# VolkmannB/bayesian-inference-with-explicit-and-implicit-prior-knowledge

Measured on AMD Instinct MI355X. Metric: particle-steps/sec (N x (T-1) / wall), SingleMassOscillator PGAS conditional-SMC sweep, higher is better.
Workload: dtype f64; 1 GPU; SingleMassOscillator PGAS sweep, nx=2, M=41 Hilbert basis (BASELINE.json configs[1]), N=1048576 particles/GPU, T=2000, fp64; particles_per_gpu=1048576, particles_total=1048576, T=2000, partition=single GPU, launch=every sweep enqueued launch by launch, verified=not checked in this run (--full checks the last timed sweep's traces), parallelism=1 GPU

## Files before the change

bayesian-inference-with-explicit-and-implicit-prior-knowledge_amd/_lib.py:

```python
from __future__ import annotations

import ctypes as C
import os

import numpy as np
import torch

_HERE = os.path.dirname(os.path.abspath(__file__))
LIB_PATH = os.environ.get("PGAS_HIP_LIB") or os.path.join(_HERE, "libpgas_hip.so")

_dp = C.POINTER(C.c_double)
_ip = C.POINTER(C.c_int32)


class PgasError(RuntimeError):
    pass


class _ModelDesc(C.Structure):
    _fields_ = [
        ("N", C.c_int32), ("T", C.c_int32), ("nx", C.c_int32), ("ny", C.c_int32), ("nu", C.c_int32),
        ("M", C.c_int32), ("D", C.c_int32),
        ("idx", _ip), ("sel", _ip), ("alpha", _dp), ("beta", _dp), ("nrm", C.c_double),
        ("H", _dp), ("LRinv", _dp), ("cR", C.c_double),
        ("m0", _dp), ("L0", _dp), ("y", _dp), ("u", _dp),
        ("device", C.c_int32), ("keep_logw_trace", C.c_int32), ("no_fast_variant", C.c_int32),
    ]


EXPORTS = [
    "pgas_create", "pgas_destroy", "pgas_last_error", "pgas_segment_size", "pgas_set_params", "pgas_set_params_dev", "pgas_get_params", "pgas_basis_eval",
    "pgas_aux_states", "pgas_init_state", "pgas_step", "pgas_sweep", "pgas_get_traces", "pgas_last_final_index",
    "pgas_suffstats", "pgas_set_profiling", "pgas_get_profile", "pgas_set_option",
    "pgas_systematic_resample", "pgas_reconstruct_trajectory",
    "pgas_trace_layout", "pgas_trace_row",
    "pgas_shard_setup", "pgas_shard_buffers", "pgas_shard_layout", "pgas_shard_block", "pgas_shard_set_peer_block", "pgas_shard_run", "pgas_ipc_export", "pgas_ipc_open",
    "pgas_hip_runtime_version", "pgas_shard_unique_id", "pgas_shard_comm_init", "pgas_shard_sweep", "pgas_shard_set_collective", "pgas_get_launch_info", "pgas_shard_probe_collective", "pgas_detmath_eval",
    "pgas_m_rng_uniform", "pgas_m_rng_normal", "pgas_m_rng_student_t", "pgas_m_rng_student_t_host", "pgas_m_rng_chi2", "pgas_m_set_time_source", "pgas_m_rng_uniform_dev", "pgas_systematic_resample_dev", "pgas_m_mniw_solve", "pgas_m_mniw_trisolve", "pgas_m_check", "pgas_m_stats_gather_update", "pgas_m_weighted_stats",
    "pgas_m_mniw_solve_n", "pgas_m_mniw_trisolve_n", "pgas_m_stats_gather_update_n", "pgas_m_weighted_stats_n", "pgas_m_expr_eval",
    "pgas_m_rng_student_t_df", "pgas_m_mniw_draw", "pgas_m_hilbert_basis", "pgas_m_lbm_diff",
    "pgas_chains_set_params_dev", "pgas_chains_sweep", "pgas_chains_get_traces", "pgas_chains_final_index", "pgas_chains_keys",
    "pgas_chains_param_draws", "pgas_chains_suffstats", "pgas_rollout", "pgas_rollout_stats", "pgas_filter",
    "pgas_m_runs_rng_normal", "pgas_m_runs_rng_student_t", "pgas_m_runs_rng_student_t_df", "pgas_m_runs_rng_uniform", "pgas_m_runs_systematic",
    "pgas_m_runs_weighted_stats", "pgas_m_rollout", "pgas_m_rollout_stats",
]



class RolloutLatent(C.Structure):
    _fields_ = [("M", C.c_int32), ("D", C.c_int32), ("n", C.c_int32), ("feat", C.c_int32), ("sel", C.c_int32 * 4),
                ("div", C.c_double * 4), ("center", C.c_double * 4), ("L", C.c_double * 4), ("size", C.c_double * 4),
                ("idx_dev", C.c_void_p), ("A_dev", C.c_void_p), ("Lrow_dev", C.c_void_p), ("fcode_dev", C.c_void_p), ("fcode_host", C.c_void_p),
                ("f_ninstr", C.c_int32), ("reserved", C.c_int32)]


class RolloutDesc(C.Structure):
    _fields_ = [(k, C.c_int32) for k in ("K", "T", "P", "L", "nx", "nu", "ny", "n_in", "nconst", "nreg", "x0_mode", "f_ninstr", "g_ninstr", "reserved")] + \
               [("f_out", C.c_int32 * 8), ("g_out", C.c_int32 * 8), ("p0", C.c_int64)] + \
               [(k, C.c_void_p) for k in ("consts_dev", "fcode_dev", "gcode_dev", "fcode_host", "gcode_host", "inputs_dev", "seeds_dev", "Qc_dev", "x0_dev",
                                          "m0L0_dev", "out_x_dev", "out_y_dev")] + \
               [("lat", RolloutLatent * 4)]


class RolloutStatsDesc(C.Structure):
    _fields_ = [(k, C.c_void_p) for k in ("y_dev", "sum_dev", "sumsq_dev", "lpd_dev", "part_dev")] + \
               [("part_bytes", C.c_uint64), ("cR", C.c_double), ("noise", C.c_int32), ("reserved", C.c_int32), ("LR", C.c_double * 64), ("LRinv", C.c_double * 64)]


ALLGATHER_FN = C.CFUNCTYPE(C.c_int, C.c_void_p, C.c_int32, C.c_void_p)

_lib = None


def load():
    global _lib
    if _lib is not None:
        return _lib
    if not os.path.exists(LIB_PATH):
        raise PgasError(f"{LIB_PATH} not found: build it with `python __graft_entry__.py` (hipcc, gfx950); there is no CPU fallback")
    L = C.CDLL(LIB_PATH)

    class _Missing:
        restype = argtypes = None

        def __init__(self, name):
            self.name = name

        def __call__(self, *a):
            raise PgasError(f"{LIB_PATH} does not export {self.name}")

    for name in EXPORTS:
        if not hasattr(L, name):
            setattr(L, name, _Missing(name))
    vp, u64, i32, i64 = C.c_void_p, C.c_uint64, C.c_int32, C.c_int64
    L.pgas_create.restype = C.c_int
    L.pgas_create.argtypes = [C.POINTER(_ModelDesc), C.POINTER(vp)]
    L.pgas_destroy.restype = None
    L.pgas_destroy.argtypes = [vp]
    L.pgas_last_error.restype = C.c_char_p
    L.pgas_last_error.argtypes = [vp]
    L.pgas_segment_size.restype = i32
    L.pgas_set_params.restype = C.c_int
    L.pgas_set_params.argtypes = [vp, vp, _dp, _dp, C.c_double, vp]
    L.pgas_set_params_dev.restype = C.c_int
    L.pgas_set_params_dev.argtypes = [vp, vp, vp, vp]
    L.pgas_get_params.restype = C.c_int
    L.pgas_get_params.argtypes = [vp, _dp, _dp, _dp, vp]
    L.pgas_basis_eval.restype = C.c_int
    L.pgas_basis_eval.argtypes = [vp, vp, i64, i32, vp, vp]
    L.pgas_aux_states.restype = C.c_int
    L.pgas_aux_states.argtypes = [vp, vp, i32, vp, vp]
    L.pgas_init_state.restype = C.c_int
    L.pgas_init_state.argtypes = [vp, u64, _dp, vp, vp]
    L.pgas_step.restype = C.c_int
    L.pgas_step.argtypes = [vp, i32, u64, vp, vp, _dp, vp, vp, vp, vp]
    L.pgas_sweep.restype = C.c_int
    L.pgas_sweep.argtypes = [vp, u64, vp, vp, vp]
    L.pgas_get_traces.restype = C.c_int
    L.pgas_get_traces.argtypes = [vp, C.POINTER(vp), C.POINTER(vp), C.POINTER(vp), C.POINTER(vp)]
    L.pgas_last_final_index.restype = C.c_int
    L.pgas_last_final_index.argtypes = [vp, C.POINTER(i64), vp]
    L.pgas_suffstats.restype = C.c_int
    L.pgas_suffstats.argtypes = [vp, vp, vp, vp, vp, vp]
    L.pgas_set_profiling.restype = C.c_int
    L.pgas_set_profiling.argtypes = [vp, i32]
    L.pgas_get_profile.restype = C.c_int
    L.pgas_get_profile.argtypes = [vp, C.POINTER(i64), C.POINTER(C.c_double), C.POINTER(i64), C.POINTER(C.c_double), vp]
    L.pgas_set_option.restype = C.c_int
    L.pgas_set_option.argtypes = [vp, i32, i64]
    L.pgas_systematic_resample.restype = C.c_int
    L.pgas_systematic_resample.argtypes = [vp, C.c_double, vp, vp, vp]
    L.pgas_reconstruct_trajectory.restype = C.c_int
    L.pgas_reconstruct_trajectory.argtypes = [vp, vp, vp, i32, i32, i64, vp, vp]
    L.pgas_shard_setup.restype = C.c_int
    L.pgas_shard_setup.argtypes = [vp, i32, i32]
    L.pgas_shard_buffers.restype = C.c_int
    L.pgas_shard_buffers.argtypes = [vp, C.POINTER(vp), C.POINTER(i64)]
    L.pgas_shard_layout.restype = C.c_int
    L.pgas_shard_layout.argtypes = [vp, i32, C.POINTER(i64)]
    L.pgas_shard_block.restype = C.c_int
    L.pgas_shard_block.argtypes = [vp, i32, i32, C.POINTER(vp), C.POINTER(i64)]
    L.pgas_shard_set_peer_block.restype = C.c_int
    L.pgas_shard_set_peer_block.argtypes = [vp, i32, i32, i32, vp]
    L.pgas_trace_layout.restype = C.c_int
    L.pgas_trace_layout.argtypes = [vp, i32, C.POINTER(i64)]
    L.pgas_trace_row.restype = C.c_int
    L.pgas_trace_row.argtypes = [vp, i32, i32, C.POINTER(vp)]
    L.pgas_shard_run.restype = C.c_int
    L.pgas_shard_run.argtypes = [vp, i32, i32, i32, u64, vp, vp, vp]
    L.pgas_shard_unique_id.restype = C.c_int
    L.pgas_shard_unique_id.argtypes = [C.c_char_p]
    L.pgas_shard_comm_init.restype = C.c_int
    L.pgas_shard_comm_init.argtypes = [vp, C.c_char_p]
    L.pgas_shard_sweep.restype = C.c_int
    L.pgas_shard_sweep.argtypes = [vp, u64, vp, vp, i32, vp]
    L.pgas_shard_set_collective.restype = C.c_int
    L.pgas_shard_set_collective.argtypes = [vp, ALLGATHER_FN, vp]
    L.pgas_detmath_eval.restype = C.c_int
    L.pgas_detmath_eval.argtypes = [i32, i32, vp, vp, vp, i64, vp, vp, vp, vp]
    L.pgas_shard_probe_collective.restype = C.c_int
    L.pgas_shard_probe_collective.argtypes = [vp, i32, vp]
    L.pgas_get_launch_info.restype = C.c_int
    L.pgas_get_launch_info.argtypes = [vp, C.POINTER(i32)]
    L.pgas_ipc_export.restype = C.c_int
    L.pgas_ipc_export.argtypes = [vp, i32, i32, C.c_char_p]
    L.pgas_hip_runtime_version.restype = C.c_int32
    L.pgas_hip_runtime_version.argtypes = []
    L.pgas_ipc_open.restype = C.c_int
    L.pgas_ipc_open.argtypes = [vp, C.c_char_p, C.POINTER(vp)]
    u32 = C.c_uint32
    L.pgas_m_rng_uniform.restype = C.c_double
    L.pgas_m_rng_uniform.argtypes = [u64, u32, u32]
    L.pgas_m_rng_normal.restype = C.c_int
    L.pgas_m_rng_normal.argtypes = [vp, u64, u32, u32, i64, i64, i32, vp, vp]
    L.pgas_m_rng_student_t.restype = C.c_int
    L.pgas_m_rng_student_t.argtypes = [vp, u64, u32, u32, i64, i64, vp, vp, vp]
    L.pgas_m_rng_student_t_host.restype = C.c_int
    L.pgas_m_rng_student_t_host.argtypes = [u64, u32, u32, i64, i64, _dp, _dp]
    L.pgas_m_set_time_source.restype = C.c_int
    L.pgas_m_set_time_source.argtypes = [vp, vp]
    L.pgas_m_rng_uniform_dev.restype = C.c_int
    L.pgas_m_rng_uniform_dev.argtypes = [vp, u64, u32, u32, vp, vp]
    L.pgas_systematic_resample_dev.restype = C.c_int
    L.pgas_systematic_resample_dev.argtypes = [vp, vp, vp, vp, vp]
    L.pgas_m_rng_chi2.restype = C.c_int
    L.pgas_m_rng_chi2.argtypes = [vp, u64, u32, u32, i64, i64, vp, vp, vp]
    L.pgas_m_mniw_solve.restype = C.c_int
    L.pgas_m_mniw_solve.argtypes = [vp, i64, i32, C.c_double, vp, vp, vp, vp, vp, vp, vp, vp, vp, vp, vp, vp, vp, vp]
    L.pgas_m_mniw_trisolve.restype = C.c_int
    L.pgas_m_mniw_trisolve.argtypes = [vp, i64, i32, vp, vp, vp, vp, vp, vp]
    L.pgas_m_rng_student_t_df.restype = C.c_int
    L.pgas_m_rng_student_t_df.argtypes = [vp, u64, C.c_uint32, C.c_uint32, i64, i64, vp, vp, C.c_double, C.c_double, vp, vp]
    L.pgas_m_mniw_draw.restype = C.c_int
    L.pgas_m_mniw_draw.argtypes = [vp, i64, C.c_double, vp, vp, vp, vp, vp, vp, C.c_double, C.c_double, vp, vp, vp]
    L.pgas_m_lbm_diff.restype = C.c_int
    L.pgas_m_lbm_diff.argtypes = [vp, i64, i32, vp, vp, vp, vp, vp, vp, C.c_double, C.c_double, vp, vp, vp, vp]
    L.pgas_m_hilbert_basis.restype = C.c_int
    L.pgas_m_hilbert_basis.argtypes = [vp, i64, i32, i32, vp, i32, vp, i32, C.POINTER(i32), _dp, _dp, _dp, _dp, vp, vp, vp]
    L.pgas_m_expr_eval.restype = C.c_int
    L.pgas_m_expr_eval.argtypes = [vp, i64, vp, i32, vp, i32, i32, i32, C.POINTER(i32), i32, vp, i32, vp, vp, i32, C.POINTER(vp), C.POINTER(i32), i32, i32,
                                   vp, vp, C.c_double, vp, vp]
    L.pgas_m_mniw_solve_n.restype = C.c_int
    L.pgas_m_mniw_solve_n.argtypes = [vp, i64, i32, i32, C.c_double, vp, vp, vp, vp, vp, vp, vp, vp, vp, vp, vp, vp, vp, vp]
    L.pgas_m_mniw_trisolve_n.restype = C.c_int
# ... 155 lines not shown
    def get_params(self):
        LS, LSinv, cS = np.zeros((self.nx, self.nx)), np.zeros((self.nx, self.nx)), C.c_double()
        self._chk(self.lib.pgas_get_params(self._h, _hp(LS), _hp(LSinv), C.byref(cS), self._stream()), "pgas_get_params")
        return LS, LSinv, float(cS.value)

    def basis_eval(self, x, t):
        x = self._dev(x).reshape(-1, self.nx)
        phi = torch.empty((x.shape[0], self.M), dtype=torch.float64, device=self.device)
        self._chk(self.lib.pgas_basis_eval(self._h, x.data_ptr(), x.shape[0], t, phi.data_ptr(), self._stream()), "pgas_basis_eval")
        return phi

    def aux_states(self, x, t):
        x = self._dev(x, shape=(self.N, self.nx))
        aux = torch.empty_like(x)
        self._chk(self.lib.pgas_aux_states(self._h, x.data_ptr(), t, aux.data_ptr(), self._stream()), "pgas_aux_states")
        return aux

    def init_state(self, seed, ref0):
        x0 = torch.empty((self.N, self.nx), dtype=torch.float64, device=self.device)
        r = _f64(ref0).reshape(self.nx)
        self._chk(self.lib.pgas_init_state(self._h, seed, _hp(r), x0.data_ptr(), self._stream()), "pgas_init_state")
        torch.cuda.current_stream(self.device).synchronize()
        return x0

    def step(self, t, seed, log_weights, state, ref_t):
        x = self._dev(state, shape=(self.N, self.nx))
        lw = None if log_weights is None else self._dev(log_weights, shape=(self.N,))
        r = _f64(ref_t.detach().cpu() if isinstance(ref_t, torch.Tensor) else ref_t).reshape(self.nx)
        lw_new = torch.empty(self.N, dtype=torch.float64, device=self.device)
        x_new = torch.empty((self.N, self.nx), dtype=torch.float64, device=self.device)
        anc = torch.empty(self.N, dtype=torch.int32, device=self.device)
        self._chk(
            self.lib.pgas_step(self._h, t, seed, None if lw is None else lw.data_ptr(), x.data_ptr(), _hp(r), lw_new.data_ptr(),
                               x_new.data_ptr(), anc.data_ptr(), self._stream()),
            "pgas_step",
        )
        torch.cuda.current_stream(self.device).synchronize()
        return lw_new, x_new, anc

    def sweep(self, seed, ref_state):
        ref = self._dev(ref_state, shape=(self.T, self.nx))
        traj = torch.empty((self.T, self.nx), dtype=torch.float64, device=self.device)
        self._chk(self.lib.pgas_sweep(self._h, seed, ref.data_ptr(), traj.data_ptr(), self._stream()), "pgas_sweep")
        self._ref_keepalive = ref
        return traj

    TRACE_X, TRACE_LA, TRACE_H, TRACE_LN, TRACE_ANC = range(5)

    def trace_layout(self, kind):
        v = (C.c_int64 * 4)()
        self._chk(self.lib.pgas_trace_layout(self._h, int(kind), v), "pgas_trace_layout")
        return tuple(int(x) for x in v)

    def trace_row(self, kind, t):
        p = C.c_void_p()
        self._chk(self.lib.pgas_trace_row(self._h, int(kind), int(t), C.byref(p)), "pgas_trace_row")
        return int(p.value)

    def traces_blocks(self, kind, row_shape, dtype):
        rows, rpb, nblk, _ = self.trace_layout(kind)
        return [self.dev_tensor(self.trace_row(kind, b * rpb), (min(rpb, rows - b * rpb),) + tuple(row_shape), dtype) for b in range(nblk)]

    def traces(self, copy_blocks=True):
        px, pa, pl, pt = C.c_void_p(), C.c_void_p(), C.c_void_p(), C.c_void_p()
        if self.trace_layout(self.TRACE_X)[2] == 1 and self.trace_layout(self.TRACE_ANC)[2] == 1:
            px.value, pa.value = self.trace_row(self.TRACE_X, 0), self.trace_row(self.TRACE_ANC, 0)
            X = torch.as_tensor(_DevView(px.value, (self.T, self.N, self.nx), "<f8", self), device=self.device)
            A = torch.as_tensor(_DevView(pa.value, (max(self.T - 1, 1), self.N), "<i4", self), device=self.device)
        elif copy_blocks:
            X = torch.cat(self.traces_blocks(self.TRACE_X, (self.N, self.nx), torch.float64))
            A = torch.cat(self.traces_blocks(self.TRACE_ANC, (self.N,), torch.int32))
        else:
            X = A = None
        self._chk(self.lib.pgas_get_traces(self._h, None, None, C.byref(pl), C.byref(pt)), "pgas_get_traces")
        Lw = torch.as_tensor(_DevView(pl.value, (self.N,), "<f8", self), device=self.device)
        Lt = torch.as_tensor(_DevView(pt.value, (self.T, self.N), "<f8", self), device=self.device) if pt.value else None
        return X, A, Lw, Lt

    def last_final_index(self):
        v = C.c_int64()
        self._chk(self.lib.pgas_last_final_index(self._h, C.byref(v), self._stream()), "pgas_last_final_index")
        return int(v.value)

    def set_profiling(self, on):
        self._chk(self.lib.pgas_set_profiling(self._h, int(on)), "pgas_set_profiling")

    def profile(self):
        n, ms, pn, pm = C.c_int64(), C.c_double(), C.c_int64(), C.c_double()
        self._chk(self.lib.pgas_get_profile(self._h, C.byref(n), C.byref(ms), C.byref(pn), C.byref(pm), self._stream()), "pgas_get_profile")
        return int(n.value), float(ms.value), int(pn.value), float(pm.value)

    def set_option(self, option, value):
        self._chk(self.lib.pgas_set_option(self._h, int(option), int(value)), "pgas_set_option")

    _utility = {}

    @classmethod
    def utility(cls, N, device=None):
        from .descriptors import BasisMap, GaussianLikelihood, HilbertBasis

        dev = torch.device("cuda", torch.cuda.current_device()) if device is None else torch.device(device)
        key = (dev.index or 0, int(N))
        if key not in cls._utility:
            basis = HilbertBasis(np.array([[1]], dtype=np.int32), np.array([[-1.0, 1.0]]))
            cls._utility[key] = cls(int(N), np.zeros((1, 1)), None, np.zeros(1), np.eye(1), GaussianLikelihood(np.eye(1), np.eye(1)),
                                    BasisMap(basis, [0]), device=dev)
        return cls._utility[key]

    def systematic_resample(self, u, logw):
        lw = self._dev(logw, shape=(self.N,))
        idx = torch.empty(self.N, dtype=torch.int32, device=self.device)
        if isinstance(u, torch.Tensor):
            self._chk(self.lib.pgas_systematic_resample_dev(self._h, u.data_ptr(), lw.data_ptr(), idx.data_ptr(), self._stream()), "pgas_systematic_resample_dev")
        else:
            self._chk(self.lib.pgas_systematic_resample(self._h, float(u), lw.data_ptr(), idx.data_ptr(), self._stream()), "pgas_systematic_resample")
        return idx

    def reconstruct_trajectory(self, particles, ancestry, idx):
        P = particles if isinstance(particles, torch.Tensor) else torch.as_tensor(np.asarray(particles, dtype=np.float64))
        P = P.to(device=self.device, dtype=torch.float64)
        if P.dim() == 2:
            P = P.unsqueeze(-1)
        P = P.contiguous()
        T, N, nx = P.shape
        if N != self.N:
            raise ValueError(f"particle count {N} does not match the context ({self.N})")
        A = ancestry if isinstance(ancestry, torch.Tensor) else torch.as_tensor(np.asarray(ancestry))
        A = A.to(device=self.device, dtype=torch.int32).contiguous()
        traj = torch.empty((T, nx), dtype=torch.float64, device=self.device)
        self._chk(self.lib.pgas_reconstruct_trajectory(self._h, P.data_ptr(), A.data_ptr(), T, nx, int(idx), traj.data_ptr(), self._stream()),
                  "pgas_reconstruct_trajectory")
        return traj

    def shard_setup(self, rank, world):
        self._chk(self.lib.pgas_shard_setup(self._h, rank, world), "pgas_shard_setup")
        self.rank, self.world = rank, world

    def shard_buffers(self):
        out = (C.c_void_p * 17)()
        sz = (C.c_int64 * 3)()
        self._chk(self.lib.pgas_shard_buffers(self._h, out, sz), "pgas_shard_buffers")
        return [int(p or 0) for p in out], tuple(int(v) for v in sz)

    def shard_layout(self, which):
        v = (C.c_int64 * 2)()
        self._chk(self.lib.pgas_shard_layout(self._h, int(which), v), "pgas_shard_layout")
        return int(v[0]), int(v[1])

    def shard_block(self, which, blk):
        p, n = C.c_void_p(), C.c_int64()
        self._chk(self.lib.pgas_shard_block(self._h, int(which), int(blk), C.byref(p), C.byref(n)), "pgas_shard_block")
        return int(p.value), int(n.value)

    def shard_set_peer_block(self, peer, which, blk, ptr):
        self._chk(self.lib.pgas_shard_set_peer_block(self._h, int(peer), int(which), int(blk), C.c_void_p(int(ptr))), "pgas_shard_set_peer_block")

    def shard_run(self, phase, t=0, t_aux=0, seed=0, ref=None, traj=None):
        self._chk(
            self.lib.pgas_shard_run(self._h, phase, t, t_aux, seed, None if ref is None else ref.data_ptr(),
                                    None if traj is None else traj.data_ptr(), self._stream()),
            "pgas_shard_run",
        )

    def shard_unique_id(self):
        buf = C.create_string_buffer(128)
        rc = self.lib.pgas_shard_unique_id(buf)
# ... 455 lines not shown
```

bayesian-inference-with-explicit-and-implicit-prior-knowledge_amd/csrc/pgas_api.hip:

```cpp
#include <hip/hip_runtime.h>
#include <hip/hip_ext.h>
#include <dlfcn.h>
#include <rccl/rccl.h>

#include <algorithm>
#include <cmath>
#include <cstdio>
#include <cstdlib>
#include <cstring>
#include <string>
#include <vector>

#include "../../include/pgas_hip.h"
#include "pgas_kernels.hip.h"
#include "pgas_resample.hip.h"
#include "pgas_suffstats.hip.h"
#include "pgas_marginal.hip.h"
#include "pgas_marginal_runs.hip.h"
#include "pgas_chains.hip.h"
#include "pgas_rollout.hip.h"
#include "pgas_rollout_stats.hip.h"
#include "pgas_filter.hip.h"
#include "../../include/pgas_marginal.h"
#include "pgas_marginal_rollout.hip.h"
// ... 230 lines not shown
    int force_slow = 0;
    int tail_groups = 0;
    int ev_stride = 8;
    int local_groups = 0;
    int overlap = 1;
    int prop_lds = 0;
    hipStream_t sB = nullptr;
    std::vector<hipEvent_t> ev_chunk;
    hipEvent_t ev_start = nullptr, ev_done = nullptr;
    double* d_phi = nullptr;
    double* d_syrk_ws = nullptr;
    size_t phi_bytes = 0, syrk_ws_bytes = 0;
    int syrk_splits = 0;
    bool peer_access_tried = false;
    const uint32_t* t_dev = nullptr;
    int max_lead = 0;
    std::vector<hipEvent_t> ev_bdone;
    int profiling = 0;
    int prof_stride = 16;
    std::vector<hipEvent_t> ev;
    std::vector<hipEvent_t> evp;
    int evp_used = 0;
    int ev_used = 0;
    int ch_cap = 0;
    int ch_params = 0;
    int ch_swept = 0;
    TransParams* ch_tp = nullptr;
    double* ch_G = nullptr;
    SweepParams* ch_sp = nullptr;
    double* ch_ures = nullptr;
    double* ch_uanc = nullptr;
    double* ch_x = nullptr;
    int32_t* ch_anc = nullptr;
    double* ch_logw = nullptr;
    UpperHdr* ch_hdr = nullptr;
    double* ch_znoise = nullptr;
    int ro_cap = 0;
    TransParams* ro_tp = nullptr;
    double* ro_G = nullptr;
    double* ro_S0 = nullptr;
    double* ro_part = nullptr;
    size_t ro_part_cap = 0;
    int fl_cap = 0;
    TransParams* fl_tp = nullptr;
    double* fl_G = nullptr;
    std::string err;
};

#define FAIL(ctx, code, ...)                                  \
    do {                                                      \
        char buf_[512];                                       \
        snprintf(buf_, sizeof buf_, __VA_ARGS__);             \
        (ctx)->err = buf_;                                    \
        return (code);                                        \
    } while (0)

#define HIPCHK(ctx, call)                                                                       \
    do {                                                                                        \
        hipError_t e_ = (call);                                                                 \
        if (e_ != hipSuccess) FAIL(ctx, e_ == hipErrorOutOfMemory ? PGAS_E_NOMEM : PGAS_E_HIP,  \
                                   "%s failed: %s", #call, hipGetErrorString(e_));              \
    } while (0)

#define KCHK(ctx, name)                                                                        \
    do {                                                                                        \
        hipError_t e_ = hipGetLastError();                                                      \
        if (e_ != hipSuccess) FAIL(ctx, PGAS_E_HIP, "launch of %s failed: %s", name, hipGetErrorString(e_)); \
    } while (0)

static int alloc_scanbufs(pgas_ctx* c, ScanBufs* sb) {
    const size_t np = (size_t)c->md.nseg * PGAS_SEG;
    const int nsegp = (c->md.nseg + 63) / 64 * 64;
    sb->nsegp = nsegp;
    HIPCHK(c, hipMalloc(&sb->laux, np * sizeof(double)));
    HIPCHK(c, hipMalloc(&sb->c1, np * sizeof(uint64_t)));
    HIPCHK(c, hipMalloc(&sb->c2, np * sizeof(uint64_t)));
    HIPCHK(c, hipMalloc(&sb->segk_w, 2 * nsegp * sizeof(double)));
    HIPCHK(c, hipMalloc(&sb->segs_w, 2 * nsegp * sizeof(uint64_t)));
    HIPCHK(c, hipMalloc(&sb->tab_e, 2 * nsegp * sizeof(double)));
    HIPCHK(c, hipMalloc(&sb->tab_sc, 2 * nsegp * sizeof(double)));
    HIPCHK(c, hipMalloc(&sb->tab_m, 2 * nsegp * sizeof(double)));
    HIPCHK(c, hipMalloc(&sb->grp_K, 2 * PG_MAX_GRP * sizeof(double)));
    HIPCHK(c, hipMalloc(&sb->grp_T, 2 * PG_MAX_GRP * sizeof(double)));
    HIPCHK(c, hipMalloc(&sb->grp_cnt, PG_MAX_GRP * sizeof(unsigned)));
    HIPCHK(c, hipMemset(sb->grp_cnt, 0, PG_MAX_GRP * sizeof(unsigned)));
    HIPCHK(c, hipMalloc(&sb->hdr, sizeof(UpperHdr)));
    HIPCHK(c, hipMemset(sb->hdr, 0, sizeof(UpperHdr)));
    sb->segk = sb->segk_w;
    sb->segs = sb->segs_w;
    sb->nseg_l = 0x40000000;
    sb->rank_stride = 0;
    sb->nsegp_g = nsegp;
    return PGAS_OK;
}
static void chains_release(pgas_ctx* c) {
    hipFree(c->ch_tp); hipFree(c->ch_G); hipFree(c->ch_sp); hipFree(c->ch_ures); hipFree(c->ch_uanc); hipFree(c->ch_x); hipFree(c->ch_anc);
    hipFree(c->ch_logw); hipFree(c->ch_hdr); hipFree(c->ch_znoise);
    c->ch_tp = nullptr; c->ch_G = nullptr; c->ch_sp = nullptr; c->ch_ures = nullptr; c->ch_uanc = nullptr; c->ch_x = nullptr; c->ch_anc = nullptr;
    c->ch_logw = nullptr; c->ch_hdr = nullptr; c->ch_znoise = nullptr;
    c->ch_cap = c->ch_params = c->ch_swept = 0;
}
static void rollout_release(pgas_ctx* c) {
    hipFree(c->ro_tp); hipFree(c->ro_G); hipFree(c->ro_S0);
    c->ro_tp = nullptr; c->ro_G = nullptr; c->ro_S0 = nullptr;
    c->ro_cap = 0;
}
static void rollout_part_release(pgas_ctx* c) {
    hipFree(c->ro_part);
    c->ro_part = nullptr;
    c->ro_part_cap = 0;
}
static void filter_release(pgas_ctx* c) {
    hipFree(c->fl_tp); hipFree(c->fl_G);
    c->fl_tp = nullptr; c->fl_G = nullptr;
    c->fl_cap = 0;
}
static void free_scanbufs(ScanBufs* sb) {
    hipFree(sb->laux); hipFree(sb->c1); hipFree(sb->c2); hipFree(sb->segk_w); hipFree(sb->segs_w);
    hipFree(sb->tab_e); hipFree(sb->tab_sc); hipFree(sb->tab_m); hipFree(sb->grp_K); hipFree(sb->grp_T); hipFree(sb->grp_cnt); hipFree(sb->hdr);
    *sb = ScanBufs{};
}

extern "C" {

int32_t pgas_segment_size(void) { return PGAS_SEG; }

const char* pgas_last_error(const pgas_ctx* ctx) { return ctx ? ctx->err.c_str() : g_create_error.c_str(); }

static int create_impl(const pgas_model_desc* d, pgas_ctx* c) {
    if (!d->idx || !d->sel || !d->alpha || !d->beta || !d->H || !d->LRinv || !d->m0 || !d->L0 || !d->y)
        FAIL(c, PGAS_E_ARG, "pgas_create: NULL table pointer");
    if (d->N < 1 || d->T < 1 || d->M < 1) FAIL(c, PGAS_E_ARG, "pgas_create: N, T, M must be >= 1");
    if (d->nx < 1 || d->nx > 2) FAIL(c, PGAS_E_ARG, "pgas_create: nx = %d not supported (compiled for nx in {1,2})", d->nx);
    if (d->ny < 1 || d->ny > PGAS_MAX_NY) FAIL(c, PGAS_E_ARG, "pgas_create: ny = %d not supported (1..%d)", d->ny, PGAS_MAX_NY);
    if (d->nu < 0 || d->nu > PGAS_MAX_NU) FAIL(c, PGAS_E_ARG, "pgas_create: nu = %d not supported (0..%d)", d->nu, PGAS_MAX_NU);
    if (d->D < 1 || d->D > PGAS_MAX_D) FAIL(c, PGAS_E_ARG, "pgas_create: D = %d not supported (1..%d)", d->D, PGAS_MAX_D);
    if (d->nu > 0 && !d->u) FAIL(c, PGAS_E_ARG, "pgas_create: nu > 0 but u == NULL");
    const int64_t nseg64 = ((int64_t)d->N + PGAS_SEG - 1) / PGAS_SEG;
    if (nseg64 > PG_MAX_NSEG) FAIL(c, PGAS_E_ARG, "pgas_create: N = %d exceeds %d particles per device", d->N, PG_MAX_NSEG * PGAS_SEG);

    DevModel& md = c->md;
    md.N = d->N; md.T = d->T; md.nx = d->nx; md.ny = d->ny; md.nu = d->nu; md.D = d->D; md.M = d->M;
    md.nseg = (int)nseg64;
    md.p0 = 0; md.Ng = d->N; md.nseg_g = md.nseg;
    c->peers = Peers{}; c->peers.world = 1; c->peers.nseg_l = md.nseg; c->peers.Nl = d->N;
    md.nrm = d->nrm; md.cR = d->cR;
    for (int k = 0; k < d->D; ++k) {
        if (d->sel[k] < 0 || d->sel[k] >= d->nx + d->nu) FAIL(c, PGAS_E_ARG, "pgas_create: sel[%d] = %d out of range", k, d->sel[k]);
        md.sel[k] = d->sel[k]; md.alpha[k] = d->alpha[k]; md.beta[k] = d->beta[k];
        int lo = d->idx[k], hi = d->idx[k], second = 0;
        for (int m = 0; m < d->M; ++m) {
            const int j = d->idx[m * d->D + k];
            if (j < 1) FAIL(c, PGAS_E_ARG, "pgas_create: idx[%d][%d] = %d must be >= 1", m, k, j);
            lo = j < lo ? j : lo; hi = j > hi ? j : hi;
        }
        for (int m = 0; m < d->M; ++m) {
            const int j = d->idx[m * d->D + k];
            if (j > lo && (second == 0 || j < second)) second = j;
        }
        md.j0[k] = lo; md.jstep[k] = second ? second - lo : 1;
        for (int m = 0; m < d->M; ++m)
            if ((d->idx[m * d->D + k] - lo) % md.jstep[k]) FAIL(c, PGAS_E_ARG, "pgas_create: idx column %d is not an arithmetic progression", k);
        md.J[k] = (hi - lo) / md.jstep[k] + 1;
        if (md.J[k] > PGAS_MAX_J) FAIL(c, PGAS_E_ARG, "pgas_create: %d frequencies in dimension %d (max %d)", md.J[k], k, PGAS_MAX_J);
    }
    for (int j = 0; j < d->ny; ++j)
        for (int k = 0; k < d->nx; ++k) md.H[j * d->nx + k] = d->H[j * d->nx + k];
    for (int j = 0; j < d->ny * d->ny; ++j) md.LRinv[j] = d->LRinv[j];
    bool fast = !d->no_fast_variant;
    for (int k = 0; k < d->D; ++k) fast = fast && md.sel[k] == k && md.jstep[k] == md.j0[k];
    if (!pick_variant(d->nx, d->D, md.J[d->D - 1], fast, md.J[0], &c->var, &md.JP))
        FAIL(c, PGAS_E_ARG, "pgas_create: innermost basis dimension has %d frequencies (compiled up to 16)", md.J[d->D - 1]);
    c->var_P = c->var.P;
    c->back = d->nx == 1 ? k_back<1> : k_back<2>;
    c->back_corrected = d->nx == 1 ? k_back_corrected<1> : k_back_corrected<2>;
    c->init = d->nx == 1 ? k_init<1> : k_init<2>;
    c->basis = d->nx == 1 ? k_basis_eval<1> : k_basis_eval<2>;
    c->keep_logw = d->keep_logw_trace;

    c->device = d->device;
    std::vector<int32_t> pos(d->M);
    int64_t gsize = 1;
    for (int k = 0; k < d->D; ++k) gsize *= (k == d->D - 1 && d->D > 1) ? md.JP : md.J[k];
    for (int m = 0; m < d->M; ++m) {
        int64_t p = 0;
        for (int k = 0; k < d->D; ++k) {
            const int ext = (k == d->D - 1 && d->D > 1) ? md.JP : md.J[k];
            p = p * ext + (d->idx[m * d->D + k] - md.j0[k]) / md.jstep[k];
        }
        pos[m] = (int32_t)p;
    }
    if (d->D == 3 && md.J[1] <= 12) {
        std::vector<uint64_t> qd((size_t)md.J[0], 0ull);
        std::vector<int> ql((size_t)md.J[0] * md.J[1], 0);
        for (int m = 0; m < d->M; ++m) {
            const int a = (d->idx[m * 3 + 0] - md.j0[0]) / md.jstep[0], b = (d->idx[m * 3 + 1] - md.j0[1]) / md.jstep[1];
            const int q = (d->idx[m * 3 + 2] - md.j0[2]) / md.jstep[2] + 1;
            if (q > ql[(size_t)a * md.J[1] + b]) ql[(size_t)a * md.J[1] + b] = q;
        }
        for (int a = 0; a < md.J[0]; ++a)
            for (int b = 0; b < md.J[1]; ++b) qd[a] |= (uint64_t)ql[(size_t)a * md.J[1] + b] << (5 * b);
        HIPCHK(c, hipMalloc(&c->d_qdesc, qd.size() * sizeof(uint64_t)));
// ... 226 lines not shown
        std::vector<const void*> h(entries, nullptr);
        for (int r = 0; r < c->world; ++r) {
            const auto& bx = c->peer_blk[r][PG_RB_X];
            const auto& ba = c->peer_blk[r][PG_RB_ANC];
            for (size_t b = 0; b < bx.size(); ++b) h[((size_t)r * 2) * nb + b] = bx[b];
            for (size_t b = 0; b < ba.size(); ++b) h[((size_t)r * 2 + 1) * nb + b] = ba[b];
        }
        HIPCHK(c, hipStreamSynchronize(st));
        if (c->d_bt_entries != entries) {
            hipFree(c->d_bt);
            c->d_bt = nullptr; c->d_bt_entries = 0;
            HIPCHK(c, hipMalloc(&c->d_bt, entries * sizeof(void*)));
            c->d_bt_entries = entries;
        }
        HIPCHK(c, hipMemcpy(c->d_bt, h.data(), entries * sizeof(void*), hipMemcpyHostToDevice));
        c->bt_dirty = false;
    }
    out->blk = c->d_bt;
    out->nblk_max = nb;
    out->shift_x = c->rs[PG_RB_X].shift;
    out->shift_anc = c->rs[PG_RB_ANC].shift;
    out->entries = (int32_t)entries;
    return PGAS_OK;
}

static int launch_backtrace(pgas_ctx* c, const UpperHdr* hdr, double* traj_dev, hipStream_t st) {
    BtTab tab;
    int rc = upload_bt_table(c, st, &tab);
    if (rc) return rc;
    const size_t lds = tab.entries <= PG_BT_TAB_LDS ? (size_t)tab.entries * sizeof(void*) : 0;
    if (c->world > 1) hipLaunchKernelGGL(k_backtrace<true>, dim3(1), dim3(PG_BT_THREADS), lds, st, c->md.N, c->md.T, c->md.nx, tab, hdr, traj_dev);
    else hipLaunchKernelGGL(k_backtrace<false>, dim3(1), dim3(PG_BT_THREADS), lds, st, c->md.N, c->md.T, c->md.nx, tab, hdr, traj_dev);
    KCHK(c, "k_backtrace");
    return PGAS_OK;
}

static int launch_groups(pgas_ctx* c, const ScanBufs& sb, int ncdf, hipStream_t st) {
    const int n1 = (c->md.nseg_g + PG_GRP - 1) / PG_GRP;
    hipLaunchKernelGGL(k_groups, dim3((n1 * ncdf + 3) / 4), dim3(256), 0, st, c->md.nseg_g, ncdf, sb);
    KCHK(c, "k_groups");
    return PGAS_OK;
}

static int launch_count(pgas_ctx* c, const ScanBufs& sb, int parity, int what, double u, hipStream_t st) {
    hipLaunchKernelGGL(k_count, dim3(1), dim3(PG_BLK), 0, st, c->md.Ng, c->md.nseg_g, sb, peers_for(c, parity), what, u, what == 1 ? (const SweepParams*)c->d_sp : (const SweepParams*)nullptr);
    KCHK(c, "k_count");
    return PGAS_OK;
}

static bool sweep_is_local(const pgas_ctx* c) { return c->local_groups && c->world == 1 && !c->sharded && c->md.nseg_g <= PG_LOCAL_NSEG && !c->force_slow; }

static bool sweep_tail_groups(const pgas_ctx* c) { return !c->sharded && c->world == 1 && c->tail_groups; }

static int launch_step(pgas_ctx* c, int t, bool local, hipStream_t st, hipEvent_t e0, hipEvent_t e1) {
    const DevModel& md = c->md;
    const int N = md.N, T = md.T;
    StepArgs ar;
    ar.t = t;
    ar.mode = (t < T ? PG_RS_SCAN : 0) | (t > 1 ? PG_RS_SEARCH : 0);
    ar.sp = c->d_sp;
    ar.u_res = c->d_ures;
    ar.u_anc = c->d_uanc;
    ar.la_t = t < T ? (const double*)c->rs[PG_RB_LA].row(t) : (const double*)nullptr;
    ar.h_t = t < T ? (const double*)c->rs[PG_RB_H].row(t) : (const double*)nullptr;
    ar.ln_prev = (const double*)c->rs[PG_RB_LN].row(t - 1);
    ar.anc_in = AncIn{};
    ar.anc_in.has_prev = t > 2 ? 1 : 0;
    if (t > 1)
        for (int r = 0; r < c->world; ++r) {
            ar.anc_in.la_s[r] = (const double*)peer_row(c, r, PG_RB_LA, t - 1);
            ar.anc_in.h_s[r] = (const double*)peer_row(c, r, PG_RB_H, t - 1);
            if (t > 2) {
                ar.anc_in.ln_p[r] = (const double*)peer_row(c, r, PG_RB_LN, t - 2);
                ar.anc_in.la_p[r] = (const double*)peer_row(c, r, PG_RB_LA, t - 2);
                ar.anc_in.anc_p[r] = (const int32_t*)peer_row(c, r, PG_RB_ANC, t - 3);
            }
        }
    ar.anc_out = t > 1 ? (int32_t*)c->rs[PG_RB_ANC].row(t - 2) : (int32_t*)nullptr;
    ar.logw_out = t == T ? c->logw_last : ((c->logw_trace && t > 1) ? c->logw_trace + (size_t)(t - 1) * N : (double*)nullptr);
    const ScanBufs& sp = c->sb[(t - 1) & 1];
    const ScanBufs& sn = c->sb[t & 1];
    const Peers pr = peers_for(c, (t - 1) & 1);
    auto kern = local ? k_step<PG_WM_LOCAL, false> : (sweep_tail_groups(c) ? k_step<PG_WM_GROUPS, true> : k_step<PG_WM_GROUPS, false>);
    if (e0 || e1) hipExtLaunchKernelGGL(kern, dim3(md.nseg + 1), dim3(PG_BLK), 0, st, e0, e1, 0, md, ar, sp, sn, pr);
    else hipLaunchKernelGGL(kern, dim3(md.nseg + 1), dim3(PG_BLK), 0, st, md, ar, sp, sn, pr);
    KCHK(c, "k_step");
    return PGAS_OK;
}

int pgas_step(pgas_ctx* c, int32_t t, uint64_t seed, const double* logw_dev, const double* x_dev, const double* ref_t_host,
              double* logw_new_dev, double* x_new_dev, int32_t* anc_dev, void* stream) {
    if (!c) return PGAS_E_ARG;
    if (!x_dev || !ref_t_host || !logw_new_dev || !x_new_dev || !anc_dev) FAIL(c, PGAS_E_ARG, "pgas_step: NULL argument");
    if (t < 0 || t >= c->md.T) FAIL(c, PGAS_E_ARG, "pgas_step: t = %d outside [0, %d)", t, c->md.T);
    if (!c->have_params) FAIL(c, PGAS_E_STATE, "pgas_step: call pgas_set_params first");
    if (c->sharded) FAIL(c, PGAS_E_STATE, "pgas_step: not available on a shard context");
    DeviceGuard guard(c->device);
    hipStream_t st = (hipStream_t)stream;
    const DevModel& md = c->md;
    install_own_peers(c);
    HIPCHK(c, hipMemcpyAsync(c->d_ref, ref_t_host, md.nx * sizeof(double), hipMemcpyHostToDevice, st));
    if (c->corrected && !c->aux_buf) HIPCHK(c, hipMalloc(&c->aux_buf, (size_t)md.N * md.nx * sizeof(double)));
    hipLaunchKernelGGL(c->var.front, dim3(md.nseg), dim3(PG_BLK), 0, st, md, (const TransParams*)c->d_tp, t, seed, x_dev, logw_dev, c->d_ref, c->corrected,
                       c->corrected ? c->aux_buf : x_new_dev, c->sb[0]);
    KCHK(c, "k_front");
    int rc = launch_groups(c, c->sb[0], 2, st);
    if (rc) return rc;
    rc = launch_count(c, c->sb[0], 0, 0, pgas_rng_uniform(seed, PGAS_STREAM_ANCESTOR, (uint32_t)t), st);
    if (rc) return rc;
    const Peers pr = peers_for(c, 0);
    if (c->corrected) {
        hipLaunchKernelGGL(c->back_corrected, dim3(md.nseg), dim3(PG_BLK), 0, st, md, (const TransParams*)c->d_tp, t, seed,
                           pgas_rng_uniform(seed, PGAS_STREAM_RESAMPLE, (uint32_t)t), c->aux_buf, c->d_ref, c->sb[0], pr, anc_dev, x_new_dev, logw_new_dev);
    } else {
        hipLaunchKernelGGL(c->back, dim3(md.nseg), dim3(PG_BLK), 0, st, md, t,
                           pgas_rng_uniform(seed, PGAS_STREAM_RESAMPLE, (uint32_t)t), x_new_dev, c->sb[0], pr, anc_dev, logw_new_dev);
    }
    KCHK(c, "k_back");
    return PGAS_OK;
}

static int alloc_rows(pgas_ctx* c, RowStore* s, int rows, size_t row_bytes, size_t block_bytes) {
    s->release();
    s->rows = rows; s->row_bytes = row_bytes;
    if (block_bytes == 0) {
        s->contiguous = true; s->shift = 30; s->nblk = 1;
        void* p = nullptr;
        HIPCHK(c, hipMalloc(&p, (size_t)rows * row_bytes));
        s->own.push_back(p);
        s->blk.push_back((char*)p);
        return PGAS_OK;
    }
    if (row_bytes > block_bytes) FAIL(c, PGAS_E_ARG, "trace rows of %zu bytes do not fit blocks of %zu bytes", row_bytes, block_bytes);
    int shift = 0;
    while (shift < 30 && ((size_t)2 << shift) * row_bytes <= block_bytes) ++shift;
    s->contiguous = false; s->shift = shift; s->nblk = (rows + (1 << shift) - 1) >> shift;
    for (int b = 0; b < s->nblk; ++b) {
        void* p = nullptr;
        HIPCHK(c, hipMalloc(&p, (size_t)s->rows_in_block(b) * row_bytes));
        s->own.push_back(p);
        s->blk.push_back((char*)p);
    }
    return PGAS_OK;
}

static int ensure_traces(pgas_ctx* c, bool blocked) {
    if (c->have_traces) return PGAS_OK;
    const DevModel& md = c->md;
    const size_t np = (size_t)md.nseg * PGAS_SEG;
    const size_t bb = c->trace_block_bytes ? c->trace_block_bytes : (blocked ? PG_TRACE_BLOCK_BYTES : 0);
    int rc = alloc_rows(c, &c->rs[PG_RB_X], md.T, (size_t)md.N * md.nx * sizeof(double), bb);
    if (!rc) rc = alloc_rows(c, &c->rs[PG_RB_ANC], md.T > 1 ? md.T - 1 : 1, (size_t)md.N * sizeof(int32_t), bb);
    for (int k : {PG_RB_LA, PG_RB_H, PG_RB_LN})
        if (!rc) rc = alloc_rows(c, &c->rs[k], md.T, np * sizeof(double), bb);
    if (rc) {
        for (RowStore& r : c->rs) r.release();
        return rc;
    }
    HIPCHK(c, hipMalloc(&c->logw_last, (size_t)md.N * sizeof(double)));
    if (c->keep_logw) {
        HIPCHK(c, hipMalloc(&c->logw_trace, (size_t)md.T * md.N * sizeof(double)));
        HIPCHK(c, hipMemset(c->logw_trace, 0, (size_t)md.T * md.N * sizeof(double)));
    }
    c->have_traces = true;
    install_own_peers(c);
    return PGAS_OK;
}

// ... 275 lines not shown
            if (!c->d_duo) HIPCHK(c, hipMalloc(&c->d_duo, sizeof(DuoShared)));
            HIPCHK(c, hipMemsetAsync(c->d_duo, 0, 64, st));
            hipLaunchKernelGGL(c->var.duo[nri], dim3(2), dim3(PG_BLK), lds, st, md, (const TransParams*)c->d_tp, (const double*)c->d_G, (const SweepParams*)c->d_sp,
                               (const double*)c->d_ures, (const double*)c->d_uanc, (const double*)c->d_m0L0, ref_dev, (double*)c->rs[PG_RB_X].blk[0],
                               (int32_t*)c->rs[PG_RB_ANC].blk[0], c->logw_last, c->logw_trace, c->sb[T & 1].hdr, traj_dev, (const double*)c->d_znoise, c->d_duo);
            KCHK(c, "k_sweep_duo");
            c->last_small = 1;
            c->last_chunk = 1;
            return PGAS_OK;
        }
        hipLaunchKernelGGL(c->var.chains[nri], dim3(1), dim3(PG_BLK), lds, st, md, (const TransParams*)c->d_tp, (const double*)c->d_G, (int64_t)c->gtotal,
                           (const SweepParams*)c->d_sp, (const double*)c->d_ures, (const double*)c->d_uanc, (const double*)c->d_m0L0, ref_dev,
                           (double*)c->rs[PG_RB_X].blk[0], (int32_t*)c->rs[PG_RB_ANC].blk[0], c->logw_last, c->sb[T & 1].hdr, traj_dev, (const double*)c->d_znoise);
        KCHK(c, "k_sweep_chains");
        c->last_small = 1;
        c->last_chunk = 1;
        return PGAS_OK;
    }
    const int chunk = c->prop_chunk > 0 ? c->prop_chunk : (c->overlap ? 1 : T);
    c->last_chunk = chunk;
    const int key[6] = {chunk, c->overlap, c->ev_stride, sweep_is_local(c) ? 1 : (sweep_tail_groups(c) ? 2 : 0), c->prop_lds, c->keep_logw};
    const bool want_graph = c->use_graph == 1 || (c->use_graph < 0 && md.N <= PG_GRAPH_AUTO_N);
    if (want_graph && !c->profiling && c->max_lead == 0 && sweep_graph_ready(c, key, chunk)) {
        const size_t nb = (size_t)T * nx * sizeof(double);
        HIPCHK(c, hipEventRecord(c->ev_g0, st));
        HIPCHK(c, hipStreamWaitEvent(c->sG, c->ev_g0, 0));
        rc = sweep_begin(c, seed, c->sG);
        if (rc) return rc;
        HIPCHK(c, hipMemcpyAsync(c->d_refbuf, ref_dev, nb, hipMemcpyDeviceToDevice, c->sG));
        HIPCHK(c, hipGraphLaunch(c->graph_exec, c->sG));
        HIPCHK(c, hipMemcpyAsync(traj_dev, c->d_trajbuf, nb, hipMemcpyDeviceToDevice, c->sG));
        HIPCHK(c, hipEventRecord(c->ev_g1, c->sG));
        HIPCHK(c, hipStreamWaitEvent(st, c->ev_g1, 0));
        c->last_graph = 1;
        return PGAS_OK;
    }
    rc = sweep_begin(c, seed, st);
    if (rc) return rc;
    return sweep_body(c, ref_dev, traj_dev, chunk, st);
}

int pgas_get_traces(pgas_ctx* c, double** x_trace, int32_t** anc_trace, double** logw_last, double** logw_trace) {
    if (!c) return PGAS_E_ARG;
    if (!c->have_traces) FAIL(c, PGAS_E_STATE, "pgas_get_traces: no sweep has run");
    if ((x_trace || anc_trace) && !c->rs[PG_RB_X].contiguous)
        FAIL(c, PGAS_E_STATE, "pgas_get_traces: this context keeps its traces in row blocks (sharded, or PGAS_OPT_TRACE_BLOCK_BYTES): use pgas_trace_layout / pgas_trace_row");
    if (x_trace) *x_trace = (double*)c->rs[PG_RB_X].blk[0];
    if (anc_trace) *anc_trace = (int32_t*)c->rs[PG_RB_ANC].blk[0];
    if (logw_last) *logw_last = c->logw_last;
    if (logw_trace) *logw_trace = c->logw_trace;
    return PGAS_OK;
}

int pgas_trace_layout(pgas_ctx* c, int32_t kind, int64_t* info4) {
    if (!c) return PGAS_E_ARG;
    if (!c->have_traces) FAIL(c, PGAS_E_STATE, "pgas_trace_layout: no traces yet (run a sweep or pgas_shard_setup first)");
    if (kind < 0 || kind >= PG_RB_NKIND || !info4) FAIL(c, PGAS_E_ARG, "pgas_trace_layout: bad argument");
    const RowStore& s = c->rs[kind];
    info4[0] = s.rows;
    info4[1] = s.contiguous ? s.rows : ((int64_t)1 << s.shift);
    info4[2] = s.nblk;
    info4[3] = (int64_t)s.row_bytes;
    return PGAS_OK;
}

int pgas_trace_row(pgas_ctx* c, int32_t kind, int32_t t, void** ptr) {
    if (!c) return PGAS_E_ARG;
    if (!c->have_traces) FAIL(c, PGAS_E_STATE, "pgas_trace_row: no traces yet");
    if (kind < 0 || kind >= PG_RB_NKIND || !ptr || t < 0 || t >= c->rs[kind < 0 || kind >= PG_RB_NKIND ? 0 : kind].rows)
        FAIL(c, PGAS_E_ARG, "pgas_trace_row: bad argument");
    *ptr = c->rs[kind].row(t);
    return PGAS_OK;
}

int pgas_last_final_index(pgas_ctx* c, int64_t* idx, void* stream) {
    if (!c) return PGAS_E_ARG;
    if (!idx) FAIL(c, PGAS_E_ARG, "pgas_last_final_index: NULL argument");
    if (!c->have_traces) FAIL(c, PGAS_E_STATE, "pgas_last_final_index: no sweep has run");
    DeviceGuard guard(c->device);
    HIPCHK(c, hipStreamSynchronize((hipStream_t)stream));
    UpperHdr h;
    HIPCHK(c, hipMemcpy(&h, c->sb[c->md.T & 1].hdr, sizeof h, hipMemcpyDeviceToHost));
    *idx = h.final_idx;
    return PGAS_OK;
}

int pgas_set_profiling(pgas_ctx* c, int32_t on) {
    if (!c) return PGAS_E_ARG;
    c->profiling = on ? 1 : 0;
    if (on > 1) c->prof_stride = on;
    if (on < 0) c->prof_stride = 1;
    return PGAS_OK;
}

int pgas_set_option(pgas_ctx* c, int32_t option, int64_t value) {
    if (!c) return PGAS_E_ARG;
    if (option == PGAS_OPT_PROPAGATE_CHUNK) {
        if (value < 0) FAIL(c, PGAS_E_ARG, "pgas_set_option: chunk must be >= 0");
        c->prop_chunk = (int)value;
        return PGAS_OK;
    }
    if (option == PGAS_OPT_FORCE_SLOW_RESAMPLE) {
        c->force_slow = value ? 1 : 0;
        return PGAS_OK;
    }
    if (option == PGAS_OPT_TAIL_GROUPS) {
        c->tail_groups = value ? 1 : 0;
        return PGAS_OK;
    }
    if (option == PGAS_OPT_MAX_LEAD) {
        if (value < 0) FAIL(c, PGAS_E_ARG, "pgas_set_option: max lead must be >= 0");
        c->max_lead = (int)value;
        return PGAS_OK;
    }
    if (option == PGAS_OPT_SYRK_SPLITS) {
        if (value < 0 || value > 32) FAIL(c, PGAS_E_ARG, "pgas_set_option: SYRK splits must be 0 (automatic) .. 32");
        c->syrk_splits = (int)value;
        return PGAS_OK;
    }
    if (option == PGAS_OPT_EVENT_STRIDE) {
        if (value < 1) FAIL(c, PGAS_E_ARG, "pgas_set_option: event stride must be >= 1");
        c->ev_stride = (int)value;
        return PGAS_OK;
    }
    if (option == PGAS_OPT_LOCAL_GROUPS) {
        c->local_groups = value ? 1 : 0;
        return PGAS_OK;
    }
    if (option == PGAS_OPT_OVERLAP) {
        c->overlap = value ? 1 : 0;
        return PGAS_OK;
    }
    if (option == PGAS_OPT_PROPAGATE_LDS) {
        if (value < 0 || value > 160 * 1024) FAIL(c, PGAS_E_ARG, "pgas_set_option: LDS bytes out of range");
        c->prop_lds = (int)value;
        return PGAS_OK;
    }
    if (option == PGAS_OPT_MFMA_PROPAGATE) {
        if (value < 0 || value > 1) FAIL(c, PGAS_E_ARG, "pgas_set_option: PGAS_OPT_MFMA_PROPAGATE takes 0 or 1");
        c->use_mx = (int)value;
        return PGAS_OK;
    }
    if (option == PGAS_OPT_SMALL_SWEEP) {
        if (value < 0 || value > 2) FAIL(c, PGAS_E_ARG, "pgas_set_option: PGAS_OPT_SMALL_SWEEP takes 0, 1 or 2");
        c->use_small = (int)value;
        return PGAS_OK;
    }
    if (option == PGAS_OPT_GRAPH) {
        c->use_graph = value ? 1 : 0;
        return PGAS_OK;
    }
    if (option == PGAS_OPT_TRACE_BLOCK_BYTES) {
        if (value < 0) FAIL(c, PGAS_E_ARG, "pgas_set_option: block bytes must be >= 0");
        if (c->have_traces) FAIL(c, PGAS_E_STATE, "pgas_set_option: the traces are already allocated");
        c->trace_block_bytes = (size_t)value;
        return PGAS_OK;
    }
    if (option == PGAS_OPT_MNIW_VALU) {
        c->mniw_valu = value == 2 ? 2 : (value ? 1 : 0);
        return PGAS_OK;
    }
    if (option == PGAS_OPT_RESAMPLE_BEFORE_PROPAGATE) {
        if (value && c->sharded) FAIL(c, PGAS_E_STATE, "pgas_set_option: the corrected mode is not available on a sharded context");
        c->corrected = value ? 1 : 0;
        return PGAS_OK;
    }
// ... 316 lines not shown

int pgas_shard_sweep(pgas_ctx* c, uint64_t seed, const double* ref_dev, double* traj_dev, int32_t propagate_chunk, void* stream) {
    if (!c) return PGAS_E_ARG;
    int rc = shard_ready(c, "pgas_shard_sweep");
    if (rc) return rc;
    if (!c->comm && !c->ag_cb) FAIL(c, PGAS_E_STATE, "pgas_shard_sweep: call pgas_shard_comm_init (RCCL) or pgas_shard_set_collective first");
    if (!ref_dev || !traj_dev) FAIL(c, PGAS_E_ARG, "pgas_shard_sweep: NULL argument");
    DeviceGuard guard(c->device);
    hipStream_t st = (hipStream_t)stream;
    const DevModel& md = c->md;
    const int T = md.T;
    rc = sweep_begin(c, seed, st);
    if (rc) return rc;
    hipLaunchKernelGGL(c->init, dim3((md.N + PG_BLK - 1) / PG_BLK), dim3(PG_BLK), 0, st, md, seed, (const SweepParams*)nullptr, c->d_m0L0, ref_dev, (double*)c->rs[PG_RB_X].row(0));
    KCHK(c, "k_init");
    c->ev_used = 0;
    c->evp_used = 0;
    if (T == 1) {
        HIPCHK(c, hipMemsetAsync(c->logw_last, 0, md.N * sizeof(double), st));
    } else {
        const int chunk = propagate_chunk > 0 ? propagate_chunk : (c->prop_chunk > 0 ? c->prop_chunk : (c->overlap ? 1 : T));
        c->last_chunk = chunk;
        rc = run_time_loop(c, ref_dev, chunk, st);
        if (rc) return rc;
    }
    rc = run_final(c, traj_dev, st);
    if (rc) return rc;
    return shard_all_gather(c, -1, st);
}

int pgas_shard_probe_collective(pgas_ctx* c, int32_t reps, void* stream) {
    if (!c) return PGAS_E_ARG;
    if (!c->sharded || !c->comm) FAIL(c, PGAS_E_STATE, "pgas_shard_probe_collective: needs an RCCL communicator (pgas_shard_comm_init)");
    if (reps < 1) FAIL(c, PGAS_E_ARG, "pgas_shard_probe_collective: reps must be >= 1");
    DeviceGuard guard(c->device);
    pgas_allgather_fn keep = c->ag_cb;
    c->ag_cb = nullptr;
    int rc = PGAS_OK;
    for (int i = 0; i < reps && rc == PGAS_OK; ++i) rc = shard_all_gather(c, 0, (hipStream_t)stream);
    c->ag_cb = keep;
    return rc;
}

int32_t pgas_hip_runtime_version(void) {
    int v = 0;
    return hipRuntimeGetVersion(&v) == hipSuccess ? v : -1;
}

int pgas_ipc_export(pgas_ctx* c, int32_t which, int32_t blk, void* handle64) {
    if (!c) return PGAS_E_ARG;
    if (!handle64) FAIL(c, PGAS_E_ARG, "pgas_ipc_export: NULL argument");
    void* p = nullptr;
    int64_t bytes = 0;
    int rc = pgas_shard_block(c, which, blk, &p, &bytes);
    if (rc) return rc;
    if (bytes >= ((int64_t)1 << 31)) FAIL(c, PGAS_E_ARG, "pgas_ipc_export: block of %lld bytes; blocks of 2 GiB and more cannot be mapped by every HIP runtime", (long long)bytes);
    static_assert(sizeof(hipIpcMemHandle_t) == 64, "handle size");
    DeviceGuard guard(c->device);
    HIPCHK(c, hipIpcGetMemHandle((hipIpcMemHandle_t*)handle64, p));
    return PGAS_OK;
}
int pgas_ipc_open(pgas_ctx* c, const void* handle64, void** ptr) {
    if (!c) return PGAS_E_ARG;
    if (!handle64 || !ptr) FAIL(c, PGAS_E_ARG, "pgas_ipc_open: NULL argument");
    DeviceGuard guard(c->device);
    if (!c->peer_access_tried) {
        c->peer_access_tried = true;
        int ndev = 0;
        if (hipGetDeviceCount(&ndev) == hipSuccess)
            for (int d = 0; d < ndev; ++d) {
                int can = 0;
                if (d != c->device && hipDeviceCanAccessPeer(&can, c->device, d) == hipSuccess && can) (void)hipDeviceEnablePeerAccess(d, 0);
            }
        (void)hipGetLastError();
    }
    hipIpcMemHandle_t h;
    memcpy(&h, handle64, sizeof h);
    HIPCHK(c, hipIpcOpenMemHandle(ptr, h, hipIpcMemLazyEnablePeerAccess));
    return PGAS_OK;
}

int pgas_detmath_eval(int32_t device, int32_t which, const double* x_dev, const double* y_dev, const uint32_t* w_dev, int64_t n, double* out0_dev,
                      double* out1_dev, uint32_t* outw_dev, void* stream) {
    if (which < 0 || which > 8 || n < 0) return PGAS_E_ARG;
    const bool words = which == 3 || which == 7;
    if (words ? !w_dev : !x_dev) return PGAS_E_ARG;
    if ((which == 5 || which == 6) && !y_dev) return PGAS_E_ARG;
    if (which == 3 ? !outw_dev : !out0_dev) return PGAS_E_ARG;
    if ((which == 2 || which == 7) && !out1_dev) return PGAS_E_ARG;
    if (n == 0) return PGAS_OK;
    DeviceGuard guard(device);
    hipLaunchKernelGGL(k_detmath, dim3((unsigned)((n + 255) / 256)), dim3(256), 0, (hipStream_t)stream, which, x_dev, y_dev, w_dev, n, out0_dev, out1_dev, outw_dev);
    return hipGetLastError() == hipSuccess ? PGAS_OK : PGAS_E_HIP;
}

static int suffstats_run(pgas_ctx* c, int C, const double* traj_dev, double* T0_dev, double* T1_dev, double* T2_dev, hipStream_t st) {
    const DevModel& md = c->md;
    DeviceGuard guard(c->device);
    const int R = md.T - 1;
    const int Mp = (md.M + md.nx + SY_BM - 1) / SY_BM * SY_BM;
    const int Rp = (R + SY_KB - 1) / SY_KB * SY_KB;
    const int nb = Mp / SY_BM, ntri = nb * (nb + 1) / 2, nkb = Rp / SY_KB;
    int S = c->syrk_splits > 0 ? c->syrk_splits : 1024 / (ntri * C);
    S = std::max(1, std::min(std::min(S, 32), nkb));
    const int kb_per_split = (nkb + S - 1) / S;
    S = (nkb + kb_per_split - 1) / kb_per_split;
    const size_t phi_need = (size_t)C * Rp * Mp * sizeof(double), ws_need = (size_t)C * S * ntri * SY_BM * SY_BM * sizeof(double);
    if (phi_need > c->phi_bytes) {
        hipFree(c->d_phi);
        c->d_phi = nullptr; c->phi_bytes = 0;
        HIPCHK(c, hipMalloc(&c->d_phi, phi_need));
        c->phi_bytes = phi_need;
    }
    if (ws_need > c->syrk_ws_bytes) {
        hipFree(c->d_syrk_ws);
        c->d_syrk_ws = nullptr; c->syrk_ws_bytes = 0;
        HIPCHK(c, hipMalloc(&c->d_syrk_ws, ws_need));
        c->syrk_ws_bytes = ws_need;
    }
    hipLaunchKernelGGL(md.nx == 1 ? k_traj_basis<1> : k_traj_basis<2>, dim3(Rp / SY_RB, 1, C), dim3(256), 0, st, md, c->d_idx, traj_dev, R, Rp, Mp, c->d_phi);
    KCHK(c, "k_traj_basis");
    hipLaunchKernelGGL(k_syrk_lds, dim3(ntri, S, C), dim3(256), 0, st, c->d_phi, Rp, Mp, kb_per_split, c->d_syrk_ws);
    KCHK(c, "k_syrk_lds");
    hipLaunchKernelGGL(k_syrk_reduce, dim3(ntri, SY_BM * SY_BM / 256, C), dim3(256), 0, st, c->d_syrk_ws, ntri, S, md.M, md.nx, T0_dev, T1_dev, T2_dev);
    KCHK(c, "k_syrk_reduce");
    return PGAS_OK;
}

int pgas_suffstats(pgas_ctx* c, const double* traj_dev, double* T0_dev, double* T1_dev, double* T2_dev, void* stream) {
    if (!c) return PGAS_E_ARG;
    if (!traj_dev || !T0_dev || !T1_dev || !T2_dev) FAIL(c, PGAS_E_ARG, "pgas_suffstats: NULL argument");
    if (c->md.T < 2) FAIL(c, PGAS_E_ARG, "pgas_suffstats: needs T >= 2");
    return suffstats_run(c, 1, traj_dev, T0_dev, T1_dev, T2_dev, (hipStream_t)stream);
}

#define PG_CHAINS_MAX 65535

static int chains_count_ok(pgas_ctx* c, int32_t C, const char* who) {
    if (C < 1 || C > PG_CHAINS_MAX) FAIL(c, PGAS_E_ARG, "%s: C = %d chains (1..%d)", who, C, PG_CHAINS_MAX);
    return PGAS_OK;
}

static int chains_sweep_ok(pgas_ctx* c, int32_t C, const char* who) {
    int rc = chains_count_ok(c, C, who);
    if (rc) return rc;
    if (c->md.N > PGAS_SEG) FAIL(c, PGAS_E_ARG, "%s: N = %d particles per chain; batched chains run one workgroup per chain, N <= %d", who, c->md.N, PGAS_SEG);
    if (c->corrected) FAIL(c, PGAS_E_ARG, "%s: the corrected mode (PGAS_OPT_RESAMPLE_BEFORE_PROPAGATE) has no batched form", who);
    if (c->keep_logw) FAIL(c, PGAS_E_ARG, "%s: keep_logw_trace has no batched form (create the context without it)", who);
    if (c->sharded) FAIL(c, PGAS_E_ARG, "%s: this context is a shard; batched chains run on an unsharded context", who);
    return PGAS_OK;
}

static int chains_alloc(pgas_ctx* c, int C) {
    if (C <= c->ch_cap) return PGAS_OK;
    chains_release(c);
    const size_t n = (size_t)C, N = c->md.N, T = c->md.T, nx = c->md.nx, anc_rows = T > 1 ? T - 1 : 1;
    const size_t per_chain = T * N * nx * sizeof(double) + T * N * 2 * sizeof(double) + anc_rows * N * sizeof(int32_t) + (size_t)c->gtotal * sizeof(double) +
                             2 * (T + 1) * sizeof(double) + N * sizeof(double) + sizeof(TransParams) + sizeof(SweepParams) + sizeof(UpperHdr);
    hipError_t e = hipSuccess;
    auto get = [&](void** p, size_t bytes) { if (e == hipSuccess) e = hipMalloc(p, bytes); };
    get((void**)&c->ch_x, n * T * N * nx * sizeof(double));
    get((void**)&c->ch_znoise, n * T * N * 2 * sizeof(double));
    get((void**)&c->ch_anc, n * anc_rows * N * sizeof(int32_t));
    get((void**)&c->ch_G, n * (size_t)c->gtotal * sizeof(double));
    get((void**)&c->ch_ures, n * (T + 1) * sizeof(double));
    get((void**)&c->ch_uanc, n * (T + 1) * sizeof(double));
    get((void**)&c->ch_logw, n * N * sizeof(double));
    get((void**)&c->ch_tp, n * sizeof(TransParams));
    get((void**)&c->ch_sp, n * sizeof(SweepParams));
    get((void**)&c->ch_hdr, n * sizeof(UpperHdr));
    if (e != hipSuccess) {
        chains_release(c);
// ... 782 lines not shown
```

bayesian-inference-with-explicit-and-implicit-prior-knowledge_amd/csrc/pgas_kernels.hip.h:

```cpp
#pragma once

#include <hip/hip_runtime.h>
#include <stdint.h>

#include "../../include/pgas_canon.h"

#define PG_BLK 256
#define PG_PPT 4
static_assert(PG_BLK * PG_PPT == PGAS_SEG && PGAS_SEG == 1024, "one workgroup owns one canonical segment of 1024 particles");
#define PG_UPPER_THREADS 256
#define PG_MAX_NSEG 8192

#ifdef PG_STAMPS
__device__ unsigned long long g_stamps[2048 * 16];
#define PG_STAMP(id)                                                                                \
    do {                                                                                            \
        if (threadIdx.x == 0) g_stamps[blockIdx.x * 16 + (id)] = __builtin_amdgcn_s_memrealtime(); \
    } while (0)
#else
#define PG_STAMP(id) do { } while (0)
#endif


#ifdef PG_NO_STREAM_STORES
// ... 58 lines not shown
#else
    return *p;
#endif
}

template <typename T>
__device__ __forceinline__ T ld_const(const T* p) {
    return *(const __attribute__((address_space(4))) T*)p;
}

struct DevModel {
    int32_t N, T, nx, ny, nu, D, M;
    int32_t J[PGAS_MAX_D], j0[PGAS_MAX_D], jstep[PGAS_MAX_D], sel[PGAS_MAX_D];
    double alpha[PGAS_MAX_D], beta[PGAS_MAX_D];
    double nrm;
    double H[PGAS_MAX_NY * 2];
    double LRinv[PGAS_MAX_NY * PGAS_MAX_NY];
    double cR;
    int32_t JP;
    int32_t nseg;
    int64_t p0;
    int32_t Ng;
    int32_t nseg_g;
    const double* y;
    const double* u;
    const uint64_t* qdesc;
};

struct TransParams {
    double LS[4], LSinv[4], cS;
    const double* G;
};

#define PGAS_LOG_2PI 0x1.d67f1c864beb4p+0

struct SweepParams {
    uint64_t seed;
    uint32_t epoch;
    uint32_t pad;
    double u_final;
};

struct UpperHdr {
    int32_t ref_idx;
    int32_t final_idx;
    unsigned long long ref_granule;
};

#define PG_MAX_RANKS 8
struct Peers {
    const uint64_t* c1[PG_MAX_RANKS];
    const uint64_t* c2[PG_MAX_RANKS];
    int32_t world, nseg_l, Nl;
};

#define PG_RB_X 0
#define PG_RB_LA 1
#define PG_RB_H 2
#define PG_RB_LN 3
#define PG_RB_ANC 4
#define PG_RB_NKIND 5
struct BtTab {
    const void* const* blk;
    int32_t nblk_max, shift_x, shift_anc, entries;
};

struct ScanBufs {
    double* laux;
    uint64_t* c1;
    uint64_t* c2;
    double* segk;
    uint64_t* segs;
    double* segk_w;
    uint64_t* segs_w;
    int32_t nseg_l;
    int32_t rank_stride;
    int32_t nsegp;
    int32_t nsegp_g;
    double* tab_e;
    double* tab_sc;
    double* tab_m;
    double* grp_K;
    double* grp_T;
    unsigned* grp_cnt;
    UpperHdr* hdr;
};

#define PG_DPP_ROW_SHR(n) (0x110 + (n))
#define PG_DPP_ROW_BCAST15 0x142
#define PG_DPP_ROW_BCAST31 0x143
template <int CTRL, int ROW_MASK>
__device__ __forceinline__ double dpp_f64(double v) {
    int lo = __double2loint(v), hi = __double2hiint(v);
    lo = __builtin_amdgcn_update_dpp(0, lo, CTRL, ROW_MASK, 0xf, true);
    hi = __builtin_amdgcn_update_dpp(0, hi, CTRL, ROW_MASK, 0xf, true);
    return __hiloint2double(hi, lo);
}
template <int CTRL, int ROW_MASK>
__device__ __forceinline__ uint64_t dpp_u64(uint64_t v) {
    int lo = (int)(uint32_t)v, hi = (int)(uint32_t)(v >> 32);
    lo = __builtin_amdgcn_update_dpp(0, lo, CTRL, ROW_MASK, 0xf, true);
    hi = __builtin_amdgcn_update_dpp(0, hi, CTRL, ROW_MASK, 0xf, true);
    return ((uint64_t)(uint32_t)hi << 32) | (uint32_t)lo;
}
__device__ __forceinline__ double readlane_f64(double v, int lane_uniform) {
    const int l = __builtin_amdgcn_readfirstlane(lane_uniform);
    return __hiloint2double(__builtin_amdgcn_readlane(__double2hiint(v), l), __builtin_amdgcn_readlane(__double2loint(v), l));
}
__device__ __forceinline__ double wave_scan_add(double v) {
    v = v + dpp_f64<PG_DPP_ROW_SHR(1), 0xf>(v);
    v = v + dpp_f64<PG_DPP_ROW_SHR(2), 0xf>(v);
    v = v + dpp_f64<PG_DPP_ROW_SHR(4), 0xf>(v);
    v = v + dpp_f64<PG_DPP_ROW_SHR(8), 0xf>(v);
    v = v + dpp_f64<PG_DPP_ROW_BCAST15, 0xa>(v);
    v = v + dpp_f64<PG_DPP_ROW_BCAST31, 0xc>(v);
    return v;
}
__device__ __forceinline__ double wave_scan_max(double v) {
    v = __builtin_fmax(v, dpp_f64<PG_DPP_ROW_SHR(1), 0xf>(v));
    v = __builtin_fmax(v, dpp_f64<PG_DPP_ROW_SHR(2), 0xf>(v));
    v = __builtin_fmax(v, dpp_f64<PG_DPP_ROW_SHR(4), 0xf>(v));
    v = __builtin_fmax(v, dpp_f64<PG_DPP_ROW_SHR(8), 0xf>(v));
    v = __builtin_fmax(v, dpp_f64<PG_DPP_ROW_BCAST15, 0xa>(v));
    v = __builtin_fmax(v, dpp_f64<PG_DPP_ROW_BCAST31, 0xc>(v));
    return v;
}
__device__ __forceinline__ uint64_t wave_incl_scan_u64(uint64_t v) {
    v += dpp_u64<PG_DPP_ROW_SHR(1), 0xf>(v);
    v += dpp_u64<PG_DPP_ROW_SHR(2), 0xf>(v);
    v += dpp_u64<PG_DPP_ROW_SHR(4), 0xf>(v);
    v += dpp_u64<PG_DPP_ROW_SHR(8), 0xf>(v);
    v += dpp_u64<PG_DPP_ROW_BCAST15, 0xa>(v);
    v += dpp_u64<PG_DPP_ROW_BCAST31, 0xc>(v);
    return v;
}
template <int CTRL, int ROW_MASK>
__device__ __forceinline__ double dpp_keep_f64(double v) {
    int lo = __double2loint(v), hi = __double2hiint(v);
    lo = __builtin_amdgcn_update_dpp(lo, lo, CTRL, ROW_MASK, 0xf, false);
    hi = __builtin_amdgcn_update_dpp(hi, hi, CTRL, ROW_MASK, 0xf, false);
    return __hiloint2double(hi, lo);
}
__device__ __forceinline__ double wave_max(double v) {
    v = __builtin_fmax(v, dpp_keep_f64<PG_DPP_ROW_SHR(1), 0xf>(v));
    v = __builtin_fmax(v, dpp_keep_f64<PG_DPP_ROW_SHR(2), 0xf>(v));
    v = __builtin_fmax(v, dpp_keep_f64<PG_DPP_ROW_SHR(4), 0xf>(v));
    v = __builtin_fmax(v, dpp_keep_f64<PG_DPP_ROW_SHR(8), 0xf>(v));
    v = __builtin_fmax(v, dpp_keep_f64<PG_DPP_ROW_BCAST15, 0xa>(v));
    v = __builtin_fmax(v, dpp_keep_f64<PG_DPP_ROW_BCAST31, 0xc>(v));
    return readlane_f64(v, 63);
}
__device__ __forceinline__ int wave_sum_i(int v) {
    v += __builtin_amdgcn_update_dpp(0, v, PG_DPP_ROW_SHR(1), 0xf, 0xf, true);
    v += __builtin_amdgcn_update_dpp(0, v, PG_DPP_ROW_SHR(2), 0xf, 0xf, true);
    v += __builtin_amdgcn_update_dpp(0, v, PG_DPP_ROW_SHR(4), 0xf, 0xf, true);
    v += __builtin_amdgcn_update_dpp(0, v, PG_DPP_ROW_SHR(8), 0xf, 0xf, true);
    v += __builtin_amdgcn_update_dpp(0, v, PG_DPP_ROW_BCAST15, 0xa, 0xf, true);
    v += __builtin_amdgcn_update_dpp(0, v, PG_DPP_ROW_BCAST31, 0xc, 0xf, true);
    return __builtin_amdgcn_readlane(v, 63);
}

template <int NX, int DSEL>
__device__ __forceinline__ double pick_input_fixed(const double (&x)[NX], const double* __restrict__ ut) {
    if constexpr (DSEL < NX) return x[DSEL];
    else return ut[DSEL - NX];
}

template <int NX>
__device__ __forceinline__ double pick_input(const DevModel& md, int d, const double (&x)[NX], const double* __restrict__ ut);
template <int NX, int DSEL, bool FAST>
__device__ __forceinline__ double basis_arg(const DevModel& md, const double (&x)[NX], const double* __restrict__ ut) {
    double v;
    if constexpr (FAST) v = pick_input_fixed<NX, DSEL>(x, ut);
    else v = pick_input<NX>(md, DSEL, x, ut);
    return PGAS_FMA(v, md.alpha[DSEL], md.beta[DSEL]);
}

template <int NX>
__device__ __forceinline__ double pick_input(const DevModel& md, int d, const double (&x)[NX], const double* __restrict__ ut) {
    const int s = md.sel[d];
    if (s == 0) return x[0];
    if (NX > 1 && s == 1) return x[NX > 1 ? 1 : 0];
    return ut[s - NX];
}

template <int NX>
__device__ __forceinline__ double loglik(const DevModel& md, const double* __restrict__ yt, const double (&xv)[NX]) {
    double e[PGAS_MAX_NY];
    double quad = 0.0;
#pragma unroll
    for (int j = 0; j < PGAS_MAX_NY; ++j) {
        e[j] = 0.0;
        if (j < md.ny) {
            e[j] = yt[j];
#pragma unroll
            for (int k = 0; k < NX; ++k) e[j] = PGAS_FMA(-md.H[j * NX + k], xv[k], e[j]);
        }
    }
#pragma unroll
    for (int j = 0; j < PGAS_MAX_NY; ++j) {
        if (j < md.ny) {
            double w = 0.0;
#pragma unroll
            for (int l = 0; l <= j; ++l) w = PGAS_FMA(md.LRinv[j * md.ny + l], e[l], w);
            quad = PGAS_FMA(w, w, quad);
        }
    }
    return PGAS_FMA(-0.5, quad, md.cR);
}

struct DimStart {
    double s0, c0, sd, cd;
};

template <int P, bool FAST = false>
__device__ __forceinline__ void dim_start_n(const DevModel& md, int d, const double (&r)[P], DimStart (&ds)[P]) {
    double a[P], sv[P], cv[P];
#pragma unroll
    for (int p = 0; p < P; ++p) a[p] = (double)md.j0[d] * r[p];
    pgas_sincospi_n(a, sv, cv, P);
#pragma unroll
    for (int p = 0; p < P; ++p) {
        ds[p].s0 = sv[p];
        ds[p].c0 = cv[p];
        ds[p].sd = sv[p];
        ds[p].cd = cv[p];
    }
    if (!FAST && md.jstep[d] != md.j0[d]) {
#pragma unroll
        for (int p = 0; p < P; ++p) a[p] = (double)md.jstep[d] * r[p];
        pgas_sincospi_n(a, sv, cv, P);
#pragma unroll
        for (int p = 0; p < P; ++p) {
            ds[p].sd = sv[p];
            ds[p].cd = cv[p];
        }
    }
}
__device__ __forceinline__ void rotate(double& sc, double& cc, double sd, double cd) {
    double sn = PGAS_FMA(sc, cd, cc * sd);
    double cn = PGAS_FMA(cc, cd, -(sc * sd));
    sc = sn;
    cc = cn;
}
#ifndef PG_QCHUNK
#define PG_QCHUNK 4
#endif
struct Cheb {
    double cur, prev, tw;
};
template <bool FAST = false>
__device__ __forceinline__ Cheb cheb_init(const DevModel& md, int d, const DimStart& ds) {
    Cheb c;
    c.cur = ds.s0;
    c.prev = (FAST || md.jstep[d] == md.j0[d]) ? 0.0 : PGAS_FMA(ds.s0, ds.cd, -(ds.c0 * ds.sd));
    c.tw = ds.cd + ds.cd;
    return c;
}
__device__ __forceinline__ void cheb_next(Cheb& c) {
    const double nx = PGAS_FMA(c.tw, c.cur, -c.prev);
    c.prev = c.cur;
    c.cur = nx;
}

template <int NX, int D, int JIN, int P, int J0T = 0, bool WIDE = false>
__device__ __forceinline__ void eval_mean(const DevModel& md, const double* __restrict__ G, const double* __restrict__ ut,
                                          const double (&x)[P][NX], double (&aux)[P][NX]) {
    constexpr bool FAST = J0T > 0;
#pragma unroll
    for (int p = 0; p < P; ++p)
#pragma unroll
        for (int k = 0; k < NX; ++k) aux[p][k] = 0.0;
    if constexpr (D == 1) {
        double r[P];
        DimStart ds[P];
#pragma unroll
        for (int p = 0; p < P; ++p) r[p] = basis_arg<NX, 0, FAST>(md, x[p], ut);
        dim_start_n<P, FAST>(md, 0, r, ds);
        const int J0 = FAST ? J0T : md.J[0];
        for (int a = 0; a < J0; ++a) {
            double g[NX];
#pragma unroll
            for (int k = 0; k < NX; ++k) g[k] = G[a * NX + k];
#pragma unroll
            for (int p = 0; p < P; ++p) {
#pragma unroll
                for (int k = 0; k < NX; ++k) aux[p][k] = PGAS_FMA(g[k], ds[p].s0, aux[p][k]);
                rotate(ds[p].s0, ds[p].c0, ds[p].sd, ds[p].cd);
            }
        }
    } else {
        constexpr int DI = D - 1;
        double tab[P][JIN];
        Cheb c0[P];
        {
            double rin[P], rout[P];
            DimStart din[P], dout[P];
#pragma unroll
            for (int p = 0; p < P; ++p) {
                rin[p] = basis_arg<NX, DI, FAST>(md, x[p], ut);
                rout[p] = basis_arg<NX, 0, FAST>(md, x[p], ut);
            }
            dim_start_n<P, FAST>(md, DI, rin, din);
            dim_start_n<P, FAST>(md, 0, rout, dout);
#pragma unroll
            for (int p = 0; p < P; ++p) {
                Cheb ci = cheb_init<FAST>(md, DI, din[p]);
#pragma unroll
                for (int q = 0; q < JIN; ++q) {
                    tab[p][q] = ci.cur;
                    cheb_next(ci);
                }
                c0[p] = cheb_init<FAST>(md, 0, dout[p]);
            }
        }
        const int J0 = FAST ? J0T : md.J[0];
        if constexpr (D == 2) {
            auto body = [&](int a) {
                double in[P][NX];
#pragma unroll
                for (int p = 0; p < P; ++p)
#pragma unroll
                    for (int k = 0; k < NX; ++k) in[p][k] = 0.0;
                const double* __restrict__ Ga = G + (size_t)a * JIN * NX;
#pragma unroll
                for (int q = 0; q < JIN; ++q) {
#pragma unroll
                    for (int k = 0; k < NX; ++k) {
                        const double g = Ga[q * NX + k];
#pragma unroll
                        for (int p = 0; p < P; ++p) in[p][k] = PGAS_FMA(g, tab[p][q], in[p][k]);
                    }
                }
#pragma unroll
                for (int p = 0; p < P; ++p) {
#pragma unroll
                    for (int k = 0; k < NX; ++k) aux[p][k] = PGAS_FMA(c0[p].cur, in[p][k], aux[p][k]);
                    cheb_next(c0[p]);
                }
            };
            if constexpr (FAST && WIDE) {
                double in[J0T][P][NX];
#pragma unroll
                for (int a = 0; a < J0T; ++a) {
                    const double* __restrict__ Ga = G + (size_t)a * JIN * NX;
#pragma unroll
                    for (int p = 0; p < P; ++p)
#pragma unroll
                        for (int k = 0; k < NX; ++k) in[a][p][k] = 0.0;
#pragma unroll
                    for (int q = 0; q < JIN; ++q)
#pragma unroll
                        for (int k = 0; k < NX; ++k)
#pragma unroll
                            for (int p = 0; p < P; ++p) in[a][p][k] = PGAS_FMA(Ga[q * NX + k], tab[p][q], in[a][p][k]);
                }
#pragma unroll
                for (int a = 0; a < J0T; ++a) {
#pragma unroll
                    for (int p = 0; p < P; ++p) {
#pragma unroll
                        for (int k = 0; k < NX; ++k) aux[p][k] = PGAS_FMA(c0[p].cur, in[a][p][k], aux[p][k]);
                        cheb_next(c0[p]);
                    }
                }
            } else if constexpr (FAST) {
                double g[JIN * NX];
#pragma unroll
                for (int i = 0; i < JIN * NX; ++i) g[i] = G[i];
#pragma unroll 1
                for (int a = 0; a < J0T; ++a) {
                    const double* __restrict__ Gn = G + (size_t)(a + 1 < J0T ? a + 1 : a) * JIN * NX;
                    double gn[JIN * NX];
#pragma unroll
                    for (int i = 0; i < JIN * NX; ++i) gn[i] = Gn[i];
                    double in[P][NX];
#pragma unroll
                    for (int p = 0; p < P; ++p)
#pragma unroll
                        for (int k = 0; k < NX; ++k) in[p][k] = 0.0;
#pragma unroll
                    for (int q = 0; q < JIN; ++q)
#pragma unroll
                        for (int k = 0; k < NX; ++k)
#pragma unroll
                            for (int p = 0; p < P; ++p) in[p][k] = PGAS_FMA(g[q * NX + k], tab[p][q], in[p][k]);
#pragma unroll
// ... 235 lines not shown
    if (i == 0) {
        TransParams tp = tp_host;
        if (S_dev != nullptr) tp_from_cov(nx, S_dev, tp);
        *tp_out = tp;
    }
}

__global__ void k_sweep_begin(uint64_t seed, uint32_t epoch, int T, SweepParams* __restrict__ sp, double* __restrict__ u_res,
                              double* __restrict__ u_anc) {
    const int t = blockIdx.x * blockDim.x + threadIdx.x;
    if (t <= T) {
        u_res[t] = pgas_rng_uniform(seed, PGAS_STREAM_RESAMPLE, (uint32_t)t);
        u_anc[t] = pgas_rng_uniform(seed, PGAS_STREAM_ANCESTOR, (uint32_t)t);
    }
    if (t == 0) {
        sp->seed = seed;
        sp->epoch = epoch;
        sp->pad = 0;
        sp->u_final = pgas_rng_uniform(seed, PGAS_STREAM_FINAL, 0u);
    }
}

template <int NX>
__global__ __launch_bounds__(PG_BLK) void k_init(DevModel md, uint64_t seed_val, const SweepParams* __restrict__ sp ,
                                                  const double* __restrict__ m0L0 ,
                                                  const double* __restrict__ ref0, double* __restrict__ x0) {
    const int64_t p = (int64_t)blockIdx.x * PG_BLK + threadIdx.x;
    if (p >= md.N) return;
    const uint64_t seed = sp ? sp->seed : seed_val;
    double z[2];
    pgas_rng_normals(seed, PGAS_STREAM_INIT, 0u, (uint64_t)(md.p0 + p), NX, z);
    double xv[NX];
#pragma unroll
    for (int k = 0; k < NX; ++k) {
        double v = m0L0[k];
#pragma unroll
        for (int l = 0; l <= k; ++l) v = PGAS_FMA(m0L0[NX + k * NX + l], z[l], v);
        xv[k] = v;
    }
    if (md.p0 + p == md.Ng - 1) {
#pragma unroll
        for (int k = 0; k < NX; ++k) xv[k] = ref0[k];
    }
    if (NX == 2 && ((uintptr_t)x0 & 15) == 0) {
        const int64_t p_wg = (int64_t)blockIdx.x * PG_BLK;
        const int64_t left = md.N - p_wg;
        st_row16<PG_ST_X>(reinterpret_cast<pg_nt_d2*>(x0) + p, x0 + p_wg * NX, 16u * threadIdx.x, pg_nt_d2{xv[0], xv[NX - 1]}, 16u * (uint32_t)(left < PG_BLK ? left : PG_BLK));
    } else {
#pragma unroll
        for (int k = 0; k < NX; ++k) st_row<PG_ST_X>(&x0[p * NX + k], xv[k]);
    }
}

template <int NB>
__device__ __forceinline__ void dev_exp_q51_n(const double (&x)[NB], uint64_t (&q)[NB]) {
    const double LOG2E = 0x1.71547652b82fep+0;
    const double LN2_HI = 0x1.62e42fefa39efp-1;
    const double LN2_LO = 0x1.abc9e3b39803fp-56;
    const double C[13] = {0x1.1eed8eff8d898p-29, 0x1.ae64567f544e4p-26, 0x1.27e4fb7789f5cp-22, 0x1.71de3a556c734p-19,
                          0x1.a01a01a01a01ap-16, 0x1.a01a01a01a01ap-13, 0x1.6c16c16c16c17p-10, 0x1.1111111111111p-7,
                          0x1.5555555555555p-5,  0x1.5555555555555p-3,  0.5, 1.0, 1.0};
    double k[NB], r[NB], p[NB];
#pragma unroll
    for (int i = 0; i < NB; ++i) {
        const double xc = __builtin_fmax(x[i], -708.0);
        k[i] = __builtin_rint(xc * LOG2E);
        r[i] = PGAS_FMA(-k[i], LN2_HI, xc);
        r[i] = PGAS_FMA(-k[i], LN2_LO, r[i]);
        p[i] = 0x1.6124613a86d09p-33;
    }
#pragma unroll
    for (int j = 0; j < 13; ++j)
#pragma unroll
        for (int i = 0; i < NB; ++i) p[i] = PGAS_FMA(p[i], r[i], C[j]);
#pragma unroll
    for (int i = 0; i < NB; ++i) {
        const int ki = (int)k[i] + PGAS_FIX_BITS;
        const double v = __hiloint2double(__double2hiint(p[i]) + (int)((unsigned)ki << 20), __double2loint(p[i]));
        const double y = v + 0x1p52;
        q[i] = ((uint64_t)(uint32_t)(__double2hiint(y) & 0x000fffff) << 32) | (uint32_t)__double2loint(y);
    }
}

#define PG_QPLANE (PG_BLK + 8)
__device__ __forceinline__ int q_slot(int i) { return (i & 3) * PG_QPLANE + (i >> 2); }
struct ScanSmem {
    uint64_t q[2][4 * PG_QPLANE];
    double red[2][PG_BLK / 64];
    uint64_t wtot[2][PG_BLK / 64];
};

template <int NW, bool STORE_B = true, bool HANDOFF = false>
__device__ __forceinline__ void segment_scan(ScanSmem& sm, const double (&lw)[NW][PG_PPT], int seg, int nsegp,
                                             uint64_t* __restrict__ cA, uint64_t* __restrict__ cB, double* __restrict__ segm,
                                             uint64_t* __restrict__ segs) {
    const int tid = threadIdx.x, lane = tid & 63, wave = tid >> 6;
    double mx[NW];
#pragma unroll
    for (int w = 0; w < NW; ++w) {
        double m = -__builtin_inf();
#pragma unroll
        for (int r = 0; r < PG_PPT; ++r) m = __builtin_fmax(m, lw[w][r]);
        m = wave_max(m);
        if (lane == 0) sm.red[w][wave] = m;
    }
    __syncthreads();
    uint64_t qsum_b = 0;
    {
#pragma unroll
        for (int w = 0; w < NW; ++w) {
            double m = sm.red[w][0];
#pragma unroll
            for (int v = 1; v < PG_BLK / 64; ++v) m = __builtin_fmax(m, sm.red[w][v]);
            const double kref = pgas_seg_ref(m);
            mx[w] = kref;
            double arg[PG_PPT];
            uint64_t qv[PG_PPT];
#pragma unroll
            for (int r = 0; r < PG_PPT; ++r) arg[r] = pgas_seg_arg(lw[w][r], kref);
            dev_exp_q51_n<PG_PPT>(arg, qv);
#pragma unroll
            for (int r = 0; r < PG_PPT; ++r) {
                if (w == 0 || STORE_B) sm.q[w][q_slot(r * PG_BLK + tid)] = qv[r];
                else qsum_b += qv[r];
            }
        }
    }
    __syncthreads();
    uint64_t loc[NW][PG_PPT], incl[NW];
#pragma unroll
    for (int w = 0; w < NW; ++w) {
        uint64_t run = 0;
        if (w == 0 || STORE_B) {
#pragma unroll
            for (int j = 0; j < PG_PPT; ++j) {
                run += sm.q[w][j * PG_QPLANE + tid];
                loc[w][j] = run;
            }
        } else {
            run = qsum_b;
        }
        incl[w] = wave_incl_scan_u64(run);
        if (lane == 63) sm.wtot[w][wave] = incl[w];
    }
    __syncthreads();
#pragma unroll
    for (int w = 0; w < NW; ++w) {
        uint64_t off = 0, tot = 0;
#pragma unroll
        for (int v = 0; v < PG_BLK / 64; ++v) {
            const uint64_t t = sm.wtot[w][v];
            if (v < wave) off += t;
            tot += t;
        }
        if (w == 0 || STORE_B) {
            const uint64_t base = off + incl[w] - loc[w][PG_PPT - 1];
            uint64_t* segc = (w == 0 ? cA : cB) + (size_t)seg * PGAS_SEG;
            pg_nt_u2* dst = reinterpret_cast<pg_nt_u2*>(segc + PG_PPT * tid);
            st_row16<PG_ST_C1>(dst, segc, 32u * tid, pg_nt_u2{base + loc[w][0], base + loc[w][1]}, PGAS_SEG * 8u);
            st_row16<PG_ST_C1>(dst + 1, segc, 32u * tid + 16u, pg_nt_u2{base + loc[w][2], base + loc[w][3]}, PGAS_SEG * 8u);
        }
        if (tid == 0) {
            if constexpr (HANDOFF) {
                __hip_atomic_store(&segm[(size_t)w * nsegp + seg], mx[w], __ATOMIC_RELAXED, __HIP_MEMORY_SCOPE_AGENT);
                __hip_atomic_store(&segs[(size_t)w * nsegp + seg], tot, __ATOMIC_RELAXED, __HIP_MEMORY_SCOPE_AGENT);
            } else {
                segm[(size_t)w * nsegp + seg] = mx[w];
                segs[(size_t)w * nsegp + seg] = tot;
            }
        }
    }
}

template <int NX, int D, int JIN, int P, int J0T = 0>
__device__ __forceinline__ void propagate_particles(const DevModel& md, const TransParams& tp, int t, uint64_t seed,
                                                    const double* __restrict__ ref_t, int seg, const double (&xprev)[PG_PPT][NX],
                                                    double (&xnew)[PG_PPT][NX], double (&la)[PG_PPT], double (&h)[PG_PPT],
                                                    double (&aux)[PG_PPT][NX]) {
    const int tid = threadIdx.x;
    const double* __restrict__ yt = md.y + (size_t)t * md.ny;
    const double* __restrict__ ut = md.u + (size_t)t * md.nu;
    double rf[NX];
#pragma unroll
    for (int k = 0; k < NX; ++k) rf[k] = ref_t[k];
#pragma unroll
    for (int r0 = 0; r0 < PG_PPT; r0 += P) {
        double xin[P][NX], ax[P][NX];
#pragma unroll
        for (int p = 0; p < P; ++p)
#pragma unroll
            for (int k = 0; k < NX; ++k) xin[p][k] = xprev[r0 + p][k];
        eval_mean<NX, D, JIN, P, J0T>(md, tp.G, ut, xin, ax);
#pragma unroll
        for (int p = 0; p < P; ++p)
#pragma unroll
            for (int k = 0; k < NX; ++k) aux[r0 + p][k] = ax[p][k];
    }
    double z0[PG_PPT], z1[PG_PPT];
    {
        pgas_u32x4 w[PG_PPT];
#pragma unroll
        for (int r = 0; r < PG_PPT; ++r) {
            const int64_t pi = (int64_t)seg * PGAS_SEG + r * PG_BLK + tid;
            w[r] = pgas_rng_block(seed, PGAS_STREAM_PROP, 0u, (uint32_t)t, (uint64_t)(md.p0 + pi));
        }
        pgas_normal_pair_n(w, z0, z1, PG_PPT);
    }
#pragma unroll
    for (int r = 0; r < PG_PPT; ++r) {
        const int64_t pi = (int64_t)seg * PGAS_SEG + r * PG_BLK + tid;
        la[r] = loglik<NX>(md, yt, aux[r]);
        double quad = 0.0;
#pragma unroll
        for (int k = 0; k < NX; ++k) {
            double w = 0.0;
#pragma unroll
            for (int l = 0; l <= k; ++l) w = PGAS_FMA(tp.LSinv[k * NX + l], rf[l] - aux[r][l], w);
            quad = PGAS_FMA(w, w, quad);
        }
        h[r] = PGAS_FMA(-0.5, quad, tp.cS);
        const double z[2] = {z0[r], z1[r]};
#pragma unroll
        for (int k = 0; k < NX; ++k) {
            double v = aux[r][k];
#pragma unroll
            for (int l = 0; l <= k; ++l) v = PGAS_FMA(tp.LS[k * NX + l], z[l], v);
            xnew[r][k] = (md.p0 + pi == md.Ng - 1) ? rf[k] : v;
        }
    }
}

template <int NX>
__device__ __forceinline__ void store_particles(const DevModel& md, double* __restrict__ x, int seg, const double (&xv)[PG_PPT][NX]) {
    const int tid = threadIdx.x;
#pragma unroll
    for (int r = 0; r < PG_PPT; ++r) {
        const int64_t pi = (int64_t)seg * PGAS_SEG + r * PG_BLK + tid;
        if (pi < md.N) {
            if constexpr (NX == 2) {
                reinterpret_cast<double2*>(x)[pi] = make_double2(xv[r][0], xv[r][1]);
            } else {
#pragma unroll
                for (int k = 0; k < NX; ++k) x[pi * NX + k] = xv[r][k];
            }
        }
    }
}

template <int NX, int D, int JIN, int P>
__device__ __forceinline__ void front_particles(const DevModel& md, const TransParams& tp, int t, uint64_t seed,
                                                const double* __restrict__ ref_t, int seg, const double (&xprev)[PG_PPT][NX],
                                                const double (&logw)[PG_PPT], int corrected, double* __restrict__ x_new,
                                                double* __restrict__ laux_out, double (&lw)[2][PG_PPT]) {
    const int tid = threadIdx.x;
    double xn[PG_PPT][NX], la[PG_PPT], h[PG_PPT], aux[PG_PPT][NX];
    propagate_particles<NX, D, JIN, P>(md, tp, t, seed, ref_t, seg, xprev, xn, la, h, aux);
    if (corrected) store_particles<NX>(md, x_new, seg, aux);
    else store_particles<NX>(md, x_new, seg, xn);
#pragma unroll
    for (int r = 0; r < PG_PPT; ++r) {
        const int64_t pi = (int64_t)seg * PGAS_SEG + r * PG_BLK + tid;
        const bool valid = pi < md.N;
        if (valid) laux_out[pi] = la[r];
        const double l1 = la[r] + logw[r];
        lw[0][r] = valid ? l1 : -__builtin_inf();
        lw[1][r] = valid ? l1 + h[r] : -__builtin_inf();
    }
}

template <int NX>
__device__ __forceinline__ void load_particles(const DevModel& md, const double* __restrict__ x, int seg, double (&xv)[PG_PPT][NX]) {
    const int tid = threadIdx.x;
#pragma unroll
    for (int r = 0; r < PG_PPT; ++r) {
        int64_t pi = (int64_t)seg * PGAS_SEG + r * PG_BLK + tid;
        if (pi >= md.N) pi = md.N - 1;
        if constexpr (NX == 2) {
            const double2 v = reinterpret_cast<const double2*>(x)[pi];
            xv[r][0] = v.x;
            xv[r][1] = v.y;
        } else {
#pragma unroll
            for (int k = 0; k < NX; ++k) xv[r][k] = x[pi * NX + k];
        }
    }
}

template <int NX, int D, int JIN, int P>
__global__ __launch_bounds__(PG_BLK) void k_front(DevModel md, const TransParams* __restrict__ tpp, int t, uint64_t seed,
                                                   const double* __restrict__ x_prev, const double* __restrict__ logw_prev,
                                                   const double* __restrict__ ref_t, int corrected, double* __restrict__ x_new, ScanBufs sb) {
    __shared__ ScanSmem sm;
    const TransParams tp = *tpp;
    const int seg = blockIdx.x, tid = threadIdx.x;
    double xv[PG_PPT][NX], lwp[PG_PPT], lw[2][PG_PPT];
    load_particles<NX>(md, x_prev, seg, xv);
#pragma unroll
    for (int r = 0; r < PG_PPT; ++r) {
        const int64_t pi = (int64_t)seg * PGAS_SEG + r * PG_BLK + tid;
        lwp[r] = (logw_prev != nullptr && pi < md.N) ? logw_prev[pi] : 0.0;
    }
    front_particles<NX, D, JIN, P>(md, tp, t, seed, ref_t, seg, xv, lwp, corrected, x_new, sb.laux, lw);
    segment_scan<2>(sm, lw, seg, sb.nsegp, sb.c1, sb.c2, sb.segk_w, sb.segs_w);
}

template <int NX, int P>
__device__ __forceinline__ void propagate_finish(const DevModel& md, const TransParams& tp, int t, uint64_t seed, const double (&rf)[NX],
                                                 const double* __restrict__ yt, int seg, int r0, const double (&aux)[P][NX],
                                                 double (&xn)[P][NX], double (&la)[P], double (&h)[P], double (&ln)[P]) {
    const int tid = threadIdx.x;
    double z0[P], z1[P];
    {
        pgas_u32x4 w[P];
#pragma unroll
        for (int p = 0; p < P; ++p) {
            const int64_t pi = (int64_t)seg * PGAS_SEG + (r0 + p) * PG_BLK + tid;
            w[p] = pgas_rng_block(seed, PGAS_STREAM_PROP, 0u, (uint32_t)t, (uint64_t)(md.p0 + pi));
        }
        pgas_normal_pair_n(w, z0, z1, P);
    }
#pragma unroll
    for (int p = 0; p < P; ++p) {
        const int64_t pi = (int64_t)seg * PGAS_SEG + (r0 + p) * PG_BLK + tid;
        la[p] = loglik<NX>(md, yt, aux[p]);
        double quad = 0.0;
#pragma unroll
        for (int k = 0; k < NX; ++k) {
            double w = 0.0;
#pragma unroll
            for (int l = 0; l <= k; ++l) w = PGAS_FMA(tp.LSinv[k * NX + l], rf[l] - aux[p][l], w);
            quad = PGAS_FMA(w, w, quad);
        }
        h[p] = PGAS_FMA(-0.5, quad, tp.cS);
        const double z[2] = {z0[p], z1[p]};
#pragma unroll
        for (int k = 0; k < NX; ++k) {
            double v = aux[p][k];
#pragma unroll
            for (int l = 0; l <= k; ++l) v = PGAS_FMA(tp.LS[k * NX + l], z[l], v);
            xn[p][k] = (md.p0 + pi == md.Ng - 1) ? rf[k] : v;
        }
        ln[p] = loglik<NX>(md, yt, xn[p]);
    }
}
template <int NX, int D, int JIN, int P, int J0T>
__device__ __forceinline__ void propagate_group(const DevModel& md, const TransParams& tp, const double* G, int t, uint64_t seed, const double (&rf)[NX],
                                                const double* __restrict__ yt, const double* __restrict__ ut, int seg, int r0,
                                                const double (&xin)[P][NX], double (&xn)[P][NX], double (&la)[P], double (&h)[P], double (&ln)[P]) {
    double aux[P][NX];
    eval_mean<NX, D, JIN, P, J0T>(md, G, ut, xin, aux);
    propagate_finish<NX, P>(md, tp, t, seed, rf, yt, seg, r0, aux, xn, la, h, ln);
}

template <int NX, int D, int JIN, int P, int J0T, int PPT, bool ONE, uint64_t MXD = 0>
__device__ __forceinline__ void propagate_kernel(const DevModel& md, const TransParams* __restrict__ tpp, const double* __restrict__ G_arg, const SweepParams* __restrict__ swp, int t0, int t1,
                                                 const double* __restrict__ x_prev , double* __restrict__ x_rows ,
                                                 const double* __restrict__ ref,
                                                 double* __restrict__ la_rows, double* __restrict__ h_rows,
                                                 double* __restrict__ ln_rows ,
                                                 const MxInfo* __restrict__ mxi = nullptr, const double* __restrict__ gimg = nullptr) {
    const int tid = threadIdx.x;
    TransParams tp;
#pragma unroll
    for (int q = 0; q < 4; ++q) {
        tp.LS[q] = ld_const(&tpp->LS[q]);
        tp.LSinv[q] = ld_const(&tpp->LSinv[q]);
    }
    tp.cS = ld_const(&tpp->cS);
    tp.G = G_arg;
    const uint64_t seed = ld_const(&swp->seed);
    const size_t row = (size_t)md.N * NX, np = (size_t)md.nseg * PGAS_SEG;
    const double* Guse = tp.G;
    double* mx_tab = nullptr;
    constexpr bool MX = MXD != 0;
    if constexpr (MX) {
        static_assert(D == 3 && P == 1, "matrix-core contraction: 3-D bases, one particle per lane and pass");
        extern __shared__ __attribute__((aligned(16))) double pg_g_lds[];
        const int nimg = ld_const(&mxi->nslots) * 64;
        for (int i = tid; i < nimg; i += PG_BLK) pg_g_lds[i] = gimg[i];
        __syncthreads();
        Guse = pg_g_lds;
        mx_tab = pg_g_lds + nimg + (tid >> 6) * (64 * PG_MX_TSTRIDE);
    } else if constexpr (D == 3) {
        extern __shared__ __attribute__((aligned(16))) double pg_g_lds[];
        const int gtot = md.J[0] * md.J[1] * JIN * NX;
        for (int i = tid; i < gtot; i += PG_BLK) pg_g_lds[i] = tp.G[i];
        __syncthreads();
        Guse = pg_g_lds;
    }
    {
        static_assert(PPT % PG_PPT == 0 && PPT % P == 0, "whole segments per workgroup, whole groups per thread");
        const int seg0 = blockIdx.x * (PPT / PG_PPT);
        auto particle = [&](int r) { return (size_t)(seg0 + r / PG_PPT) * PGAS_SEG + (size_t)(r % PG_PPT) * PG_BLK + tid; };
        auto load_state = [&](int r, double (&xr)[NX]) {
            size_t pi = particle(r);
            if (pi >= (size_t)md.N) pi = md.N - 1;
            if constexpr (NX == 2) {
#ifdef PG_NT_LOADS
                const pg_nt_d2 v = __builtin_nontemporal_load(reinterpret_cast<const pg_nt_d2*>(x_prev) + pi);
#else
                const double2 v = reinterpret_cast<const double2*>(x_prev)[pi];
#endif
                xr[0] = v.x;
                xr[1] = v.y;
            } else {
#pragma unroll
                for (int k = 0; k < NX; ++k) xr[k] = x_prev[pi * NX + k];
            }
        };
        const size_t p_wg = (size_t)seg0 * PGAS_SEG;
        const size_t left = (size_t)md.N - p_wg;
        const uint32_t x_bytes = 16u * (uint32_t)(left < (size_t)PPT * PG_BLK ? left : (size_t)PPT * PG_BLK);
        const uint32_t h_bytes = 8u * (uint32_t)(np - p_wg < (size_t)PPT * PG_BLK ? np - p_wg : (size_t)PPT * PG_BLK);
        constexpr bool kPackH = PG_ST_H_PACK && P % 2 == 0;
        (void)x_bytes; (void)h_bytes;
        double xv[ONE ? 1 : PPT][NX];
        if constexpr (!ONE) {
#pragma unroll
            for (int r = 0; r < PPT; ++r) load_state(r, xv[r]);
        }
        for (int t = t0; t < (ONE ? t0 + 1 : t1); ++t) {
            const double* __restrict__ yt = md.y + (size_t)t * md.ny;
            const double* __restrict__ ut = md.u + (size_t)t * md.nu;
            double rf[NX];
#pragma unroll
            for (int k = 0; k < NX; ++k) rf[k] = ref[(size_t)t * NX + k];
            double* __restrict__ xt = x_rows + (size_t)(t - t0) * row;
            const size_t hrow = (size_t)(t - t0) * np;
            constexpr int kUnroll = ONE ? 1 : PPT / P;
            double xnext[P][NX];
            if constexpr (ONE) {
#pragma unroll
                for (int p = 0; p < P; ++p) load_state(p, xnext[p]);
            }
// ... 227 lines not shown
```

bayesian-inference-with-explicit-and-implicit-prior-knowledge_amd/csrc/pgas_resample.hip.h:

```cpp
#pragma once

#include "pgas_kernels.hip.h"

#define PG_GRP PGAS_GRP
#define PG_MAX_GRP (PG_MAX_NSEG / PG_GRP)
#define PG_WIN_SEG 1024
#define PG_WIN_GRP (PG_WIN_SEG / PG_GRP)
#define PG_LOCAL_NSEG PG_WIN_SEG
#ifndef PG_FSTAGE
#define PG_FSTAGE 2
#endif
#define PG_NCAND 8
#define PG_DEXP_ZERO (-32768)
#ifdef PG_COLD_NOINLINE
#define PG_COLD_ATTR __noinline__
#else
#define PG_COLD_ATTR __forceinline__
#endif
static_assert(PG_MAX_GRP <= 128, "top_scan_wave handles two blocks of 64 groups");
#ifdef PG_DEBUG_DUMP
__device__ double g_dbg[4][64];
#endif

__device__ __forceinline__ size_t partial_at(const ScanBufs& sb, int cdf, int b) {
    return (size_t)(b / sb.nseg_l) * sb.rank_stride + (size_t)cdf * sb.nsegp + (size_t)(b % sb.nseg_l);
}

__device__ __forceinline__ void group_scan_wave(double kk, uint64_t ss, double& e, double& sc, double& m, double& Kg) {
    const int lane = threadIdx.x & 63;
    Kg = wave_max(kk);
    sc = pgas_lvl_scale(kk, Kg);
    const double t = sc * (pgas_u64_to_double(ss) * PGAS_FIX_INV);
    const double incl = wave_scan_add(t);
    const double up = __shfl_up(incl, 1);
    e = lane ? up : 0.0;
    m = wave_scan_max(e + t);
}

__device__ __forceinline__ double top_scan_wave(int n1, const double (&Kg)[2], const double (&Tg)[2], double (&E)[2], double (&sig)[2],
                                                double (&CM)[2]) {
    const int lane = threadIdx.x & 63;
    const double K = wave_max(__builtin_fmax(Kg[0], Kg[1]));
    double TT[2], inc[2];
#pragma unroll
    for (int h = 0; h < 2; ++h) {
        sig[h] = pgas_lvl_scale(Kg[h], K);
        TT[h] = sig[h] * Tg[h];
    }
    inc[0] = wave_scan_add(TT[0]);
    inc[1] = n1 > 64 ? wave_scan_add(TT[1]) : 0.0;
    const double BT0 = readlane_f64(inc[0], 63);
    double W[2];
#pragma unroll
    for (int h = 0; h < 2; ++h) {
        const double up = __shfl_up(inc[h], 1);
        E[h] = (h ? BT0 : 0.0) + (lane ? up : 0.0);
        W[h] = (lane + 64 * h < n1) ? E[h] + TT[h] : 0.0;
    }
    CM[0] = wave_scan_max(W[0]);
    const double M0 = readlane_f64(CM[0], 63);
    CM[1] = M0;
    double S = M0;
    if (n1 > 64) {
        CM[1] = __builtin_fmax(wave_scan_max(W[1]), M0);
        S = readlane_f64(CM[1], 63);
    }
    return S;
}

__device__ __forceinline__ int dexp_of(double sc) { return sc > 0.0 ? (int)((pgas_d2bits(sc) >> 52) & 0x7ff) - 1023 : PG_DEXP_ZERO; }
__device__ __forceinline__ double sc_of(int dexp) { return dexp == PG_DEXP_ZERO ? 0.0 : ldexp(1.0, dexp); }

struct SegParams {
    double e, sc, mp;
    double E, sg, cp;
};
__device__ __forceinline__ double num_of(uint64_t c, const SegParams& p) {
    const double v = __builtin_fmax(p.mp, p.e + p.sc * (pgas_u64_to_double(c) * PGAS_FIX_INV));
    return __builtin_fmax(p.cp, p.E + p.sg * v);
}

__device__ __forceinline__ void group_records_wave(const ScanBufs& sb, int nseg, int cdf, int g, bool coherent) {
    const int lane = threadIdx.x & 63;
    const int b = g * PG_GRP + lane;
    double kk = -__builtin_inf();
    uint64_t ss = 0;
    if (b < nseg) {
        const size_t at = partial_at(sb, cdf, b);
        if (coherent) {
            kk = __hip_atomic_load(&sb.segk[at], __ATOMIC_RELAXED, __HIP_MEMORY_SCOPE_AGENT);
            ss = __hip_atomic_load(&sb.segs[at], __ATOMIC_RELAXED, __HIP_MEMORY_SCOPE_AGENT);
        } else {
            kk = sb.segk[at];
            ss = sb.segs[at];
        }
    }
    double e, sc, m, Kg;
    group_scan_wave(kk, ss, e, sc, m, Kg);
    const int nb = nseg - g * PG_GRP < PG_GRP ? nseg - g * PG_GRP : PG_GRP;
    const double Tg = readlane_f64(m, nb - 1);
    if (b < nseg) {
        const size_t o = (size_t)cdf * sb.nsegp_g + b;
        sb.tab_e[o] = e;
        sb.tab_sc[o] = sc;
        sb.tab_m[o] = m;
    }
    if (lane == 0) {
        sb.grp_K[cdf * PG_MAX_GRP + g] = Kg;
        sb.grp_T[cdf * PG_MAX_GRP + g] = Tg;
    }
}

__global__ __launch_bounds__(256) void k_groups(int nseg, int ncdf, ScanBufs sb) {
    __builtin_amdgcn_s_setprio(3);
    const int n1 = (nseg + PG_GRP - 1) / PG_GRP;
    const int w = blockIdx.x * 4 + (threadIdx.x >> 6);
    if (w >= n1 * ncdf) return;
    group_records_wave(sb, nseg, w / n1, w % n1, false);
}

#define PG_WM_GROUPS 0
#define PG_WM_LOCAL 1
template <int LOCAL>
struct WinSmemT {
    double cm[PG_WIN_SEG];
    union {
        double num[PG_FSTAGE][PGAS_SEG];
        struct {
            double e[PG_WIN_SEG], mp[PG_WIN_SEG];
        } tab;
        ScanSmem scan;
        int a[PGAS_SEG];
    } u;
    short dexp[PG_WIN_SEG];
    double gE[PG_WIN_GRP], gS[PG_WIN_GRP], gCP[PG_WIN_GRP];
    double topCM[LOCAL ? 1 : PG_MAX_GRP], topE[LOCAL ? 1 : PG_MAX_GRP], topS[LOCAL ? 1 : PG_MAX_GRP];
    double grK[PG_WIN_GRP], grT[PG_WIN_GRP];
    int cand_b[PG_NCAND];
    double cand_cy[PG_NCAND];
    SegParams cand_p[PG_NCAND];
    double S;
    int g_lo, g_hi;
    int cnt[2];
    unsigned long long wsum[PG_BLK / 64];
};

template <int LOCAL>
__device__ __forceinline__ bool window_head(WinSmemT<LOCAL>& sm, const ScanBufs& sb, int cdf, int nseg, double U_first, double U_last,
                                            double& S, int& win_b0, int& nwin) {
    const int tid = threadIdx.x, lane = tid & 63, wave = tid >> 6;
    const int n1 = (nseg + PG_GRP - 1) / PG_GRP;
    if constexpr (LOCAL == PG_WM_LOCAL) {
        double mreg[PG_WIN_GRP / 4];
#pragma unroll
        for (int e4 = 0; e4 < PG_WIN_GRP / 4; ++e4) {
            const int g = wave + 4 * e4, b = (g << 6) + lane;
            double kk = -__builtin_inf();
            uint64_t ss = 0;
            if (b < nseg) {
                const size_t at = partial_at(sb, cdf, b);
                kk = sb.segk[at];
                ss = sb.segs[at];
            }
            double e, sc, m, Kg;
            group_scan_wave(kk, ss, e, sc, m, Kg);
            const double upm = __shfl_up(m, 1);
            sm.u.tab.e[b] = e;
            sm.u.tab.mp[b] = lane ? upm : 0.0;
            sm.dexp[b] = (short)dexp_of(sc);
            mreg[e4] = m;
            int nb = nseg - g * PG_GRP;
            nb = nb < 1 ? 1 : (nb > PG_GRP ? PG_GRP : nb);
            const double Tg = readlane_f64(m, nb - 1);
            if (lane == 0) {
                sm.grK[g] = Kg;
                sm.grT[g] = Tg;
            }
        }
        __syncthreads();
        const double Kg2[2] = {lane < n1 ? sm.grK[lane & (PG_WIN_GRP - 1)] : -__builtin_inf(), -__builtin_inf()};
        const double Tg2[2] = {lane < n1 ? sm.grT[lane & (PG_WIN_GRP - 1)] : 0.0, 0.0};
        double E[2], sig[2], CM[2];
        S = top_scan_wave(n1, Kg2, Tg2, E, sig, CM);
#pragma unroll
        for (int e4 = 0; e4 < PG_WIN_GRP / 4; ++e4) {
            const int g = wave + 4 * e4, b = (g << 6) + lane;
            const double Eg = readlane_f64(E[0], g), sg = readlane_f64(sig[0], g), cpr = readlane_f64(CM[0], g ? g - 1 : 0);
            const double cp = g ? cpr : 0.0;
            sm.cm[b] = b < nseg ? __builtin_fmax(cp, Eg + sg * mreg[e4]) : __builtin_inf();
        }
        if (wave == 0) {
            const double upc = __shfl_up(CM[0], 1);
            if (lane < PG_WIN_GRP) {
                sm.gE[lane] = E[0];
                sm.gS[lane] = sig[0];
                sm.gCP[lane] = lane ? upc : 0.0;
            }
        }
        __syncthreads();
        win_b0 = 0;
        nwin = nseg;
// ... 442 lines not shown
__global__ __launch_bounds__(PG_BLK) void k_back(DevModel md, int t, double u1, const double* __restrict__ x_cur, ScanBufs sb, Peers pr,
                                                  int32_t* __restrict__ anc_out, double* __restrict__ logw_out) {
    __shared__ WinSmemT<PG_WM_GROUPS> sm;
    const int seg = blockIdx.x, tid = threadIdx.x;
    double xv[PG_PPT][NX];
    load_particles<NX>(md, x_cur, seg, xv);
    int anc[PG_PPT];
    resample_slots<PG_WM_GROUPS>(md, sm, u1, sb, pr, seg, anc_out, anc, sb.hdr->ref_idx);
    const double* __restrict__ yt = md.y + (size_t)t * md.ny;
#pragma unroll
    for (int r = 0; r < PG_PPT; ++r) {
        const int64_t i = (int64_t)seg * PGAS_SEG + r * PG_BLK + tid;
        if (i < md.N) logw_out[i] = loglik<NX>(md, yt, xv[r]) - sb.laux[anc[r]];
    }
}

template <int NX>
__global__ __launch_bounds__(PG_BLK) void k_back_corrected(DevModel md, const TransParams* __restrict__ tpp, int t, uint64_t seed, double u1,
                                                            const double* __restrict__ aux, const double* __restrict__ ref_t, ScanBufs sb, Peers pr,
                                                            int32_t* __restrict__ anc_out, double* __restrict__ x_new,
                                                            double* __restrict__ logw_out) {
    const TransParams tp = *tpp;
    __shared__ WinSmemT<PG_WM_GROUPS> sm;
    const int seg = blockIdx.x, tid = threadIdx.x;
    int anc[PG_PPT];
    resample_slots<PG_WM_GROUPS>(md, sm, u1, sb, pr, seg, anc_out, anc, sb.hdr->ref_idx);
    const double* __restrict__ yt = md.y + (size_t)t * md.ny;
    double z0[PG_PPT], z1[PG_PPT];
    {
        pgas_u32x4 w[PG_PPT];
#pragma unroll
        for (int r = 0; r < PG_PPT; ++r) {
            const int64_t pi = (int64_t)seg * PGAS_SEG + r * PG_BLK + tid;
            w[r] = pgas_rng_block(seed, PGAS_STREAM_PROP, 0u, (uint32_t)t, (uint64_t)(md.p0 + pi));
        }
        pgas_normal_pair_n(w, z0, z1, PG_PPT);
    }
    double xn[PG_PPT][NX];
#pragma unroll
    for (int r = 0; r < PG_PPT; ++r) {
        const int64_t pi = (int64_t)seg * PGAS_SEG + r * PG_BLK + tid;
        const int src = pi < md.N ? anc[r] : 0;
        const double z[2] = {z0[r], z1[r]};
#pragma unroll
        for (int k = 0; k < NX; ++k) {
            double v = aux[(size_t)src * NX + k];
#pragma unroll
            for (int l = 0; l <= k; ++l) v = PGAS_FMA(tp.LS[k * NX + l], z[l], v);
            xn[r][k] = (md.p0 + pi == md.Ng - 1) ? ref_t[k] : v;
        }
        if (pi < md.N) logw_out[pi] = loglik<NX>(md, yt, xn[r]) - sb.laux[src];
    }
    store_particles<NX>(md, x_new, seg, xn);
}

__global__ __launch_bounds__(PG_BLK) void k_systematic(DevModel md, double u, const double* __restrict__ u_dev, ScanBufs sb, Peers pr,
                                                      int32_t* __restrict__ idx_out) {
    __shared__ WinSmemT<PG_WM_GROUPS> sm;
    int anc[PG_PPT];
    resample_slots<PG_WM_GROUPS>(md, sm, u_dev ? u_dev[0] : u, sb, pr, blockIdx.x, idx_out, anc, -1);
}

#define PG_RS_SEARCH 1
#define PG_RS_SCAN 2

struct StepArgs {
    int t, mode;
    const SweepParams* sp;
    const double* u_res;
    const double* u_anc;
    const double* la_t;
    const double* h_t;
    const double* ln_prev;
    AncIn anc_in;
    int32_t* anc_out;
    double* logw_out;
};

template <int LOCAL>
__device__ PG_COLD_ATTR int cdf_count_wg_cold(WinSmemT<LOCAL>& sm, const ScanBufs& sb, const Peers& pr, int nseg, int N, double U, const AncIn& in) {
    return cdf_count_wg<LOCAL>(sm, sb, pr, 1, nseg, N, U, nullptr, nullptr, &in);
}

#ifndef PG_STEP_OCC
#define PG_STEP_OCC 4
#endif
template <int LOCAL, bool TAIL = false>
__global__ __launch_bounds__(PG_BLK, PG_STEP_OCC) void k_step(DevModel md, StepArgs ar, ScanBufs sb_prev, ScanBufs sb_next, Peers pr) {
    __shared__ WinSmemT<LOCAL> sm;
    const int tid = threadIdx.x;
    const int N = md.N;
    const unsigned tag = ar.sp->epoch * 2654435761u + (unsigned)ar.t;
    const double u1_prev = (ar.mode & PG_RS_SEARCH) ? ar.u_res[ar.t - 1] : 0.0, u2_prev = (ar.mode & PG_RS_SEARCH) ? ar.u_anc[ar.t - 1] : 0.0;
#ifdef PG_STEP_PRIO
    __builtin_amdgcn_s_setprio(PG_STEP_PRIO);
#endif
    if (blockIdx.x == 0) {
        if (!(ar.mode & PG_RS_SEARCH)) return;
        const int r = cdf_count_wg<LOCAL>(sm, sb_prev, pr, 1, md.nseg_g, md.Ng, u2_prev, nullptr, nullptr, &ar.anc_in);
        if (tid == 0)
            __hip_atomic_store(&sb_prev.hdr->ref_granule, ((unsigned long long)tag << 32) | (unsigned)r, __ATOMIC_RELAXED,
                               __HIP_MEMORY_SCOPE_AGENT);
        return;
    }
    const int seg = blockIdx.x - 1;
    const int64_t base_i = (int64_t)seg * PGAS_SEG;
    PG_STAMP(0);
    double lnv[PG_PPT] = {0.0, 0.0, 0.0, 0.0};
    double lwp[PG_PPT] = {0.0, 0.0, 0.0, 0.0};
    int a[PG_PPT] = {0, 0, 0, 0};
    int a4[PG_PPT] = {0, 0, 0, 0};
    constexpr bool kAnc16 = PG_ST_ANC == 2;
    auto store_trace = [&]() {
        if constexpr (kAnc16) {
            const int64_t left = N - base_i;
            if (left >= PGAS_SEG && ((uintptr_t)ar.anc_out & 15) == 0) {
                typedef int pg_i32x4 __attribute__((ext_vector_type(4)));
                st_row16<PG_ST_ANC>(reinterpret_cast<pg_i32x4*>(ar.anc_out + base_i) + tid, ar.anc_out + base_i, 16u * tid, pg_i32x4{a4[0], a4[1], a4[2], a4[3]}, PGAS_SEG * 4u);
            } else {
#pragma unroll
                for (int j = 0; j < PG_PPT; ++j)
                    if (PG_PPT * tid + j < left) st_row<PG_ST_ANC>(&ar.anc_out[base_i + PG_PPT * tid + j], (int32_t)a4[j]);
            }
        } else {
#pragma unroll
            for (int j = 0; j < PG_PPT; ++j)
                if (base_i + slot_of(tid, j) < N) st_row<PG_ST_ANC>(&ar.anc_out[base_i + slot_of(tid, j)], (int32_t)a[j]);
        }
    };
    if (ar.mode & PG_RS_SEARCH) {
        resample_search<LOCAL>(md, sm, u1_prev, sb_prev, pr, seg, a, [&]() {
#pragma unroll
            for (int r = 0; r < PG_PPT; ++r) lnv[r] = ld_stream(&ar.ln_prev[(size_t)base_i + r * PG_BLK + tid]);
        });
        const bool last_wg = md.p0 + base_i + PGAS_SEG >= md.Ng;
        if (last_wg) {
            __syncthreads();
            if (tid == 0) {
                unsigned long long g = 0;
                int spins = 0;
                for (; spins < (1 << 16); ++spins) {
                    g = __hip_atomic_load(&sb_prev.hdr->ref_granule, __ATOMIC_RELAXED, __HIP_MEMORY_SCOPE_AGENT);
                    if ((unsigned)(g >> 32) == tag) break;
                    __builtin_amdgcn_s_sleep(8);
                }
                sm.cnt[1] = ((unsigned)(g >> 32) == tag) ? (int)(unsigned)g : -1;
            }
            __syncthreads();
            int ref_idx = sm.cnt[1];
            if (ref_idx < 0) {
                __syncthreads();
                ref_idx = cdf_count_wg_cold<LOCAL>(sm, sb_prev, pr, md.nseg_g, md.Ng, u2_prev, ar.anc_in);
            }
#pragma unroll
            for (int j = 0; j < PG_PPT; ++j)
                if (md.p0 + base_i + slot_of(tid, j) == md.Ng - 1) a[j] = ref_idx;
        }
        PG_STAMP(4);
        __syncthreads();
#pragma unroll
        for (int j = 0; j < PG_PPT; ++j) sm.u.a[slot_of(tid, j)] = a[j];
        __syncthreads();
        int anv[PG_PPT];
        double lav[PG_PPT];
#pragma unroll
        for (int r = 0; r < PG_PPT; ++r) anv[r] = sm.u.a[r * PG_BLK + tid];
        if constexpr (kAnc16) {
            const int2* a2 = reinterpret_cast<const int2*>(sm.u.a);
            const int2 lo = a2[2 * tid], hi = a2[2 * tid + 1];
            a4[0] = lo.x, a4[1] = lo.y, a4[2] = hi.x, a4[3] = hi.y;
        }
        if (pr.world == 1) {
            const double* __restrict__ la0 = ar.anc_in.la_s[0];
#pragma unroll
            for (int r = 0; r < PG_PPT; ++r) lav[r] = la0[anv[r]];
        } else {
            const double* rowp[PG_PPT];
            int off[PG_PPT];
#pragma unroll
            for (int r = 0; r < PG_PPT; ++r) {
                const int ra = anv[r] / pr.Nl;
                off[r] = anv[r] - ra * pr.Nl;
                rowp[r] = ar.anc_in.la_s[ra];
            }
#pragma unroll
            for (int r = 0; r < PG_PPT; ++r) lav[r] = rowp[r][off[r]];
        }
#pragma unroll
        for (int r = 0; r < PG_PPT; ++r) {
            const int64_t i = base_i + r * PG_BLK + tid;
            lwp[r] = i < N ? lnv[r] - lav[r] : 0.0;
        }
        PG_STAMP(5);
        if (ar.logw_out != nullptr) {
#pragma unroll
            for (int r = 0; r < PG_PPT; ++r) {
                const int64_t i = base_i + r * PG_BLK + tid;
                if (i < N) ar.logw_out[i] = lwp[r];
            }
        }
        __syncthreads();
    }
    if (ar.mode & PG_RS_SCAN) {
        double lw[2][PG_PPT];
        {
            double lat[PG_PPT], ht[PG_PPT];
#pragma unroll
            for (int r = 0; r < PG_PPT; ++r) {
                const size_t pi = (size_t)base_i + r * PG_BLK + tid;
                lat[r] = ld_stream(&ar.la_t[pi]);
                ht[r] = ld_stream(&ar.h_t[pi]);
            }
#pragma unroll
            for (int r = 0; r < PG_PPT; ++r) {
                const size_t pi = (size_t)base_i + r * PG_BLK + tid;
                const bool valid_p = pi < (size_t)N;
                const double l1 = lat[r] + lwp[r];
                lw[0][r] = valid_p ? l1 : -__builtin_inf();
                lw[1][r] = valid_p ? l1 + ht[r] : -__builtin_inf();
            }
        }
        PG_STAMP(6);
        segment_scan<2, false, TAIL>(sm.u.scan, lw, seg, sb_next.nsegp, sb_next.c1, sb_next.c2, sb_next.segk_w, sb_next.segs_w);
        PG_STAMP(8);
        if constexpr (TAIL) {
            if (tid < 64) {
                const int g = seg / PG_GRP;
                const int nb = md.nseg - g * PG_GRP < PG_GRP ? md.nseg - g * PG_GRP : PG_GRP;
                unsigned arrived = 0;
                if (tid == 0) {
                    asm volatile("s_waitcnt vmcnt(0)" ::: "memory");
                    arrived = __hip_atomic_fetch_add(&sb_next.grp_cnt[g], 1u, __ATOMIC_RELAXED, __HIP_MEMORY_SCOPE_AGENT);
                }
                arrived = __builtin_amdgcn_readfirstlane(arrived);
                if (arrived == (unsigned)(nb - 1)) {
                    __builtin_amdgcn_fence(__ATOMIC_ACQUIRE, "agent");
                    asm volatile("s_waitcnt vmcnt(0)" ::: "memory");
                    group_records_wave(sb_next, md.nseg, 0, g, true);
                    group_records_wave(sb_next, md.nseg, 1, g, true);
                    if (tid == 0) __hip_atomic_store(&sb_next.grp_cnt[g], 0u, __ATOMIC_RELAXED, __HIP_MEMORY_SCOPE_AGENT);
                }
            }
        }
    }
    if (ar.mode & PG_RS_SEARCH) store_trace();
    PG_STAMP(7);
}

__global__ __launch_bounds__(PG_BT_THREADS) void k_backtrace_idx(int N, int T, int nx, const double* __restrict__ x_trace, const int32_t* __restrict__ anc_trace,
                                                                 int64_t idx, double* __restrict__ traj) {
    __shared__ int32_t rec[PG_BT_CHUNK];
    const pg_gi32p anc = (pg_gi32p)anc_trace;
    const pg_gf64p x = (pg_gf64p)x_trace;
    const bool vec2 = nx == 2 && (((uintptr_t)traj | (uintptr_t)x_trace) & 15) == 0;
    auto anc_row = [&](int i) { return anc + (size_t)i * N; };
    bt_passes(T, nx, (uint32_t)idx, rec, traj, vec2,
              [&](int hi, int lo, uint32_t b, int32_t* rc) { return bt_chase_rows(hi, lo, b, rc, anc_row); },
              [&](int i, uint32_t b) { return x + ((size_t)i * N + b) * nx; });
}

__global__ void k_detmath(int which, const double* __restrict__ x, const double* __restrict__ y, const uint32_t* __restrict__ w,
                          int64_t n, double* __restrict__ o0, double* __restrict__ o1, uint32_t* __restrict__ ow) {
    const int64_t i = (int64_t)blockIdx.x * blockDim.x + threadIdx.x;
    if (i >= n) return;
    switch (which) {
    case 0: o0[i] = pgas_exp(x[i]); break;
    case 1: o0[i] = pgas_log(x[i]); break;
    case 2: pgas_sincospi(x[i], &o0[i], &o1[i]); break;
    case 3: {
        const pgas_u32x4 r = pgas_philox4x32_10(w[6 * i], w[6 * i + 1], w[6 * i + 2], w[6 * i + 3], w[6 * i + 4], w[6 * i + 5]);
        for (int k = 0; k < 4; ++k) ow[4 * i + k] = r.v[k];
        break;
    }
    case 4: o0[i] = pgas_seg_ref(x[i]); break;
    case 5: o0[i] = pgas_seg_arg(x[i], y[i]); break;
    case 6: o0[i] = pgas_lvl_scale(x[i], y[i]); break;
    case 7: {
        const pgas_u32x4 r = pgas_philox4x32_10(w[6 * i], w[6 * i + 1], w[6 * i + 2], w[6 * i + 3], w[6 * i + 4], w[6 * i + 5]);
        pgas_normal_pair(r, &o0[i], &o1[i]);
        break;
    }
    case 8: {
        const double xv[1] = {x[i]};
        uint64_t qv[1];
        dev_exp_q51_n<1>(xv, qv);
        o0[i] = (double)qv[0];
        break;
    }
    default: break;
    }
}

__device__ __forceinline__ void lds_barrier() { asm volatile("s_waitcnt lgkmcnt(0)\n\ts_barrier" ::: "memory"); }

template <int NX, int D, int JIN, int J0T>
__device__ __forceinline__ void small_particle_step(const DevModel& md, const TransParams& tp, const double* __restrict__ G, const double* __restrict__ ut,
                                                    const double* __restrict__ yt, const double (&rf)[NX], bool conditioned, const double (&xin)[1][NX],
                                                    const double (&z)[2], double (&xt)[NX], double& la, double& h, double& ln) {
    double aux[1][NX];
    eval_mean<NX, D, JIN, 1, J0T, true>(md, G, ut, xin, aux);
    la = loglik<NX>(md, yt, aux[0]);
    double quad = 0.0;
#pragma unroll
    for (int k = 0; k < NX; ++k) {
        double w = 0.0;
#pragma unroll
        for (int l = 0; l <= k; ++l) w = PGAS_FMA(tp.LSinv[k * NX + l], rf[l] - aux[0][l], w);
        quad = PGAS_FMA(w, w, quad);
    }
    h = PGAS_FMA(-0.5, quad, tp.cS);
#pragma unroll
    for (int k = 0; k < NX; ++k) {
        double v = aux[0][k];
#pragma unroll
        for (int l = 0; l <= k; ++l) v = PGAS_FMA(tp.LS[k * NX + l], z[l], v);
        xt[k] = conditioned ? rf[k] : v;
    }
    ln = loglik<NX>(md, yt, xt);
}

struct SmallSmem {
    uint64_t q[2][PGAS_SEG];
    double num[2][PGAS_SEG];
    double la[PGAS_SEG];
    double red[2][PG_BLK / 64];
    uint64_t wtot[2][PG_BLK / 64];
    int cnt[PG_BLK / 64];
};

template <int NW, int NR>
__device__ __forceinline__ void small_scan(SmallSmem& sm, const double (&lw)[NW][NR], int n, double (&S)[NW]) {
    const int tid = threadIdx.x, lane = tid & 63, wave = tid >> 6;
#pragma unroll
    for (int w = 0; w < NW; ++w) {
        double m = -__builtin_inf();
#pragma unroll
        for (int r = 0; r < NR; ++r) m = __builtin_fmax(m, lw[w][r]);
        m = wave_max(m);
        if (lane == 0) sm.red[w][wave] = m;
    }
    lds_barrier();
    uint64_t qkeep[NW] = {};
#pragma unroll
    for (int w = 0; w < NW; ++w) {
        double m = sm.red[w][0];
#pragma unroll
        for (int v = 1; v < PG_BLK / 64; ++v) m = __builtin_fmax(m, sm.red[w][v]);
        const double kref = pgas_seg_ref(m);
        double arg[NR];
        uint64_t qv[NR];
#pragma unroll
        for (int r = 0; r < NR; ++r) arg[r] = pgas_seg_arg(lw[w][r], kref);
        dev_exp_q51_n<NR>(arg, qv);
        if constexpr (NR == 1) qkeep[w] = qv[0];
        else {
#pragma unroll
            for (int r = 0; r < NR; ++r) sm.q[w][r * PG_BLK + tid] = qv[r];
        }
    }
    if constexpr (NR > 1) lds_barrier();
    uint64_t loc[NW][NR], incl[NW];
#pragma unroll
    for (int w = 0; w < NW; ++w) {
        uint64_t run = 0;
#pragma unroll
        for (int j = 0; j < NR; ++j) {
            run += NR == 1 ? qkeep[w] : sm.q[w][NR * tid + j];
            loc[w][j] = run;
        }
// ... 309 lines not shown
```

include/pgas_hip.h:

```cpp
#ifndef PGAS_HIP_H
#define PGAS_HIP_H

#include <stdint.h>

#ifdef __cplusplus
extern "C" {
#endif

#define PGAS_OK 0
#define PGAS_E_ARG (-1)
#define PGAS_E_HIP (-2)
#define PGAS_E_STATE (-3)
#define PGAS_E_NOMEM (-4)

typedef struct pgas_ctx pgas_ctx;

typedef struct pgas_model_desc {
    int32_t N;
    int32_t T;
    int32_t nx, ny, nu;
    int32_t M, D;
    const int32_t* idx;
    const int32_t* sel;
    const double* alpha;
    const double* beta;
    double nrm;
    const double* H;
    const double* LRinv;
    double cR;
    const double* m0;
    const double* L0;
    const double* y;
    const double* u;
    int32_t device;
    int32_t keep_logw_trace;
    int32_t no_fast_variant;
} pgas_model_desc;

int pgas_create(const pgas_model_desc* desc, pgas_ctx** out);
void pgas_destroy(pgas_ctx* ctx);
const char* pgas_last_error(const pgas_ctx* ctx);

int32_t pgas_segment_size(void);

int pgas_set_params(pgas_ctx* ctx, const double* A_dev, const double* LS_host, const double* LSinv_host,
                    double cS, void* stream);

int pgas_set_params_dev(pgas_ctx* ctx, const double* A_dev, const double* S_dev, void* stream);
int pgas_get_params(pgas_ctx* ctx, double* LS_host, double* LSinv_host, double* cS, void* stream);

int pgas_basis_eval(pgas_ctx* ctx, const double* x_dev, int64_t np, int32_t t, double* phi_dev, void* stream);

int pgas_aux_states(pgas_ctx* ctx, const double* x_dev, int32_t t, double* aux_dev, void* stream);

int pgas_init_state(pgas_ctx* ctx, uint64_t seed, const double* ref0_host, double* x0_dev, void* stream);

int pgas_step(pgas_ctx* ctx, int32_t t, uint64_t seed, const double* logw_dev, const double* x_dev,
              const double* ref_t_host, double* logw_new_dev, double* x_new_dev, int32_t* anc_dev, void* stream);

int pgas_sweep(pgas_ctx* ctx, uint64_t seed, const double* ref_dev, double* traj_dev, void* stream);

int pgas_get_traces(pgas_ctx* ctx, double** x_trace, int32_t** anc_trace, double** logw_last, double** logw_trace);
#define PGAS_TRACE_X 0
#define PGAS_TRACE_LA 1
#define PGAS_TRACE_H 2
#define PGAS_TRACE_LN 3
#define PGAS_TRACE_ANC 4
int pgas_trace_layout(pgas_ctx* ctx, int32_t kind, int64_t* info4);
int pgas_trace_row(pgas_ctx* ctx, int32_t kind, int32_t t, void** row_dev);

int pgas_last_final_index(pgas_ctx* ctx, int64_t* idx, void* stream);

int pgas_set_profiling(pgas_ctx* ctx, int32_t on);
int pgas_get_profile(pgas_ctx* ctx, int64_t* resample_launches, double* resample_ms, int64_t* propagate_launches,
                     double* propagate_ms, void* stream);
int pgas_get_launch_info(pgas_ctx* ctx, int32_t* info4);

#define PGAS_OPT_PROPAGATE_CHUNK 1
#define PGAS_OPT_PROPAGATE_LDS 4
#define PGAS_OPT_OVERLAP 3
#define PGAS_OPT_FORCE_SLOW_RESAMPLE 2
#define PGAS_OPT_RESAMPLE_BEFORE_PROPAGATE 5
#define PGAS_OPT_LOCAL_GROUPS 7
#define PGAS_OPT_MAX_LEAD 11
#define PGAS_OPT_SYRK_SPLITS 10
#define PGAS_OPT_TAIL_GROUPS 9
#define PGAS_OPT_EVENT_STRIDE 8
#define PGAS_OPT_SMALL_SWEEP 14
#define PGAS_OPT_MFMA_PROPAGATE 15
#define PGAS_OPT_GRAPH 13
#define PGAS_OPT_TRACE_BLOCK_BYTES 12
#define PGAS_OPT_MNIW_VALU 6
int pgas_set_option(pgas_ctx* ctx, int32_t option, int64_t value);

int pgas_systematic_resample(pgas_ctx* ctx, double u, const double* logw_dev, int32_t* idx_dev, void* stream);
int pgas_systematic_resample_dev(pgas_ctx* ctx, const double* u_dev, const double* logw_dev, int32_t* idx_dev, void* stream);
int pgas_reconstruct_trajectory(pgas_ctx* ctx, const double* x_dev, const int32_t* anc_dev, int32_t T, int32_t nx, int64_t idx,
                                double* traj_dev, void* stream);

#define PGAS_SHARD_INIT 0
#define PGAS_SHARD_PROPAGATE 1
#define PGAS_SHARD_STEP 2
#define PGAS_SHARD_GROUPS 3
#define PGAS_SHARD_FINAL_SCAN 4
#define PGAS_SHARD_FINAL 5
#define PGAS_SHARD_BACKTRACE 6
int pgas_shard_setup(pgas_ctx* ctx, int32_t rank, int32_t world);
int pgas_shard_buffers(pgas_ctx* ctx, void** out17, int64_t* sizes3);
int pgas_shard_layout(pgas_ctx* ctx, int32_t which, int64_t* info2);
int pgas_shard_block(pgas_ctx* ctx, int32_t which, int32_t blk, void** ptr_dev, int64_t* bytes);
int pgas_shard_set_peer_block(pgas_ctx* ctx, int32_t peer, int32_t which, int32_t blk, const void* ptr_dev);
int pgas_shard_run(pgas_ctx* ctx, int32_t phase, int32_t t, int32_t t_aux, uint64_t seed, const double* ref_dev, double* traj_dev,
                   void* stream);
typedef int (*pgas_allgather_fn)(void* user, int32_t parity, void* stream);
int pgas_shard_unique_id(void* id128);
int pgas_shard_comm_init(pgas_ctx* ctx, const void* id128);
int pgas_shard_set_collective(pgas_ctx* ctx, pgas_allgather_fn fn, void* user);
int pgas_shard_sweep(pgas_ctx* ctx, uint64_t seed, const double* ref_dev, double* traj_dev, int32_t propagate_chunk, void* stream);
int pgas_shard_probe_collective(pgas_ctx* ctx, int32_t reps, void* stream);
int32_t pgas_hip_runtime_version(void);

int pgas_ipc_export(pgas_ctx* ctx, int32_t which, int32_t blk, void* handle64);
int pgas_ipc_open(pgas_ctx* ctx, const void* handle64, void** ptr);

int pgas_detmath_eval(int32_t device, int32_t which, const double* x_dev, const double* y_dev, const uint32_t* w_dev, int64_t n,
                      double* out0_dev, double* out1_dev, uint32_t* outw_dev, void* stream);

int pgas_suffstats(pgas_ctx* ctx, const double* traj_dev, double* T0_dev, double* T1_dev, double* T2_dev, void* stream);


int pgas_chains_set_params_dev(pgas_ctx* ctx, int32_t C, const double* A_dev, const double* S_dev, void* stream);
int pgas_chains_sweep(pgas_ctx* ctx, int32_t C, const uint64_t* seeds_dev, const double* ref_dev, double* traj_dev, void* stream);
int pgas_chains_get_traces(pgas_ctx* ctx, double** x_trace, int32_t** anc_trace, double** logw_last);
int pgas_chains_final_index(pgas_ctx* ctx, int32_t C, int64_t* idx_host, void* stream);
int pgas_chains_keys(pgas_ctx* ctx, int32_t C, const uint64_t* keys_dev, int32_t first, uint64_t* out_dev, void* stream);
int pgas_chains_param_draws(pgas_ctx* ctx, int32_t C, const uint64_t* keys6_dev, double df, double* chi2_dev, double* normals_T_dev,
                            double* normals_A_dev, void* stream);
int pgas_chains_suffstats(pgas_ctx* ctx, int32_t C, const double* traj_dev, double* T0_dev, double* T1_dev, double* T2_dev, void* stream);

int pgas_rollout(pgas_ctx* ctx, int32_t K, int32_t P, int64_t p0, const uint64_t* seeds_dev, const double* A_dev, const double* S_dev,
                 const double* x0_dev, int32_t x0_mode, double* out_dev, void* stream);
int pgas_rollout_stats(pgas_ctx* ctx, int32_t K, int32_t P, int64_t p0, const uint64_t* seeds_dev, const double* A_dev, const double* S_dev,
                       const double* x0_dev, int32_t x0_mode, const double* LR, double* sum_dev, double* sumsq_dev, double* lpd_dev, void* stream);

int pgas_filter(pgas_ctx* ctx, int32_t K, const uint64_t* seeds_dev, const double* A_dev, const double* S_dev, const double* x0_dev,
                int32_t x0_mode, double* ell_dev, double* loglik_dev, double* ess_dev, double* pred_sum_dev, double* pred_sumsq_dev,
                double* filt_sum_dev, double* wtot_dev, double* x_dev, int32_t* anc_dev, void* stream);

#ifdef __cplusplus
}
#endif
#endif
```

Before: 35.10 billion particle-steps/s.

## Add scanner workgroups for group scan and inline custom sincospi/normal math

Swaps the last-arriver atomic counter for dedicated scanner workgroups inside k_step. Each segment publishes its max and total as tagged 32-bit halves in a hand-off buffer, and the scanner waves spin on those tags to build the group records. A scan_fail flag and a status API report a scanner that gives up after a spin limit. Separately, for the D==2 fast path, it adds hand-written sincospi, Box-Muller normal, division and sqrt routines that use rcp/rsq builtins and scalar-operand FMAs. This trades extra workgroups and spin-waiting risk for less serialized tail work and cheaper transcendental math.

```diff
diff --git a/bayesian-inference-with-explicit-and-implicit-prior-knowledge_amd/_lib.py b/bayesian-inference-with-explicit-and-implicit-prior-knowledge_amd/_lib.py
--- a/bayesian-inference-with-explicit-and-implicit-prior-knowledge_amd/_lib.py
+++ b/bayesian-inference-with-explicit-and-implicit-prior-knowledge_amd/_lib.py
@@ -30,7 +30,7 @@
 
 EXPORTS = [
     "pgas_create", "pgas_destroy", "pgas_last_error", "pgas_segment_size", "pgas_set_params", "pgas_set_params_dev", "pgas_get_params", "pgas_basis_eval",
-    "pgas_aux_states", "pgas_init_state", "pgas_step", "pgas_sweep", "pgas_get_traces", "pgas_last_final_index",
+    "pgas_aux_states", "pgas_init_state", "pgas_step", "pgas_sweep", "pgas_get_traces", "pgas_last_final_index", "pgas_scan_status",
     "pgas_suffstats", "pgas_set_profiling", "pgas_get_profile", "pgas_set_option",
     "pgas_systematic_resample", "pgas_reconstruct_trajectory",
     "pgas_trace_layout", "pgas_trace_row",
@@ -120,6 +120,8 @@
     L.pgas_get_traces.argtypes = [vp, C.POINTER(vp), C.POINTER(vp), C.POINTER(vp), C.POINTER(vp)]
     L.pgas_last_final_index.restype = C.c_int
     L.pgas_last_final_index.argtypes = [vp, C.POINTER(i64), vp]
+    L.pgas_scan_status.restype = C.c_int
+    L.pgas_scan_status.argtypes = [vp, C.POINTER(i32), vp]
     L.pgas_suffstats.restype = C.c_int
     L.pgas_suffstats.argtypes = [vp, vp, vp, vp, vp, vp]
     L.pgas_set_profiling.restype = C.c_int
@@ -441,6 +443,11 @@
         self._chk(self.lib.pgas_last_final_index(self._h, C.byref(v), self._stream()), "pgas_last_final_index")
         return int(v.value)
 
+    def scan_gave_up(self):
+        v = C.c_int32()
+        self._chk(self.lib.pgas_scan_status(self._h, C.byref(v), self._stream()), "pgas_scan_status")
+        return bool(v.value)
+
     def set_profiling(self, on):
         self._chk(self.lib.pgas_set_profiling(self._h, int(on)), "pgas_set_profiling")
 
diff --git a/bayesian-inference-with-explicit-and-implicit-prior-knowledge_amd/csrc/pgas_api.hip b/bayesian-inference-with-explicit-and-implicit-prior-knowledge_amd/csrc/pgas_api.hip
--- a/bayesian-inference-with-explicit-and-implicit-prior-knowledge_amd/csrc/pgas_api.hip
+++ b/bayesian-inference-with-explicit-and-implicit-prior-knowledge_amd/csrc/pgas_api.hip
@@ -336,8 +336,10 @@
     HIPCHK(c, hipMalloc(&sb->tab_m, 2 * nsegp * sizeof(double)));
     HIPCHK(c, hipMalloc(&sb->grp_K, 2 * PG_MAX_GRP * sizeof(double)));
     HIPCHK(c, hipMalloc(&sb->grp_T, 2 * PG_MAX_GRP * sizeof(double)));
-    HIPCHK(c, hipMalloc(&sb->grp_cnt, PG_MAX_GRP * sizeof(unsigned)));
-    HIPCHK(c, hipMemset(sb->grp_cnt, 0, PG_MAX_GRP * sizeof(unsigned)));
+    HIPCHK(c, hipMalloc(&sb->hand, (size_t)nsegp * 8 * sizeof(unsigned long long)));
+    HIPCHK(c, hipMemset(sb->hand, 0, (size_t)nsegp * 8 * sizeof(unsigned long long)));
+    HIPCHK(c, hipMalloc(&sb->scan_fail, 16));
+    HIPCHK(c, hipMemset(sb->scan_fail, 0, 16));
     HIPCHK(c, hipMalloc(&sb->hdr, sizeof(UpperHdr)));
     HIPCHK(c, hipMemset(sb->hdr, 0, sizeof(UpperHdr)));
     sb->segk = sb->segk_w;
@@ -371,7 +373,7 @@
 }
 static void free_scanbufs(ScanBufs* sb) {
     hipFree(sb->laux); hipFree(sb->c1); hipFree(sb->c2); hipFree(sb->segk_w); hipFree(sb->segs_w);
-    hipFree(sb->tab_e); hipFree(sb->tab_sc); hipFree(sb->tab_m); hipFree(sb->grp_K); hipFree(sb->grp_T); hipFree(sb->grp_cnt); hipFree(sb->hdr);
+    hipFree(sb->tab_e); hipFree(sb->tab_sc); hipFree(sb->tab_m); hipFree(sb->grp_K); hipFree(sb->grp_T); hipFree(sb->hand); hipFree(sb->scan_fail); hipFree(sb->hdr);
     *sb = ScanBufs{};
 }
 
@@ -764,8 +766,9 @@
     const ScanBufs& sn = c->sb[t & 1];
     const Peers pr = peers_for(c, (t - 1) & 1);
     auto kern = local ? k_step<PG_WM_LOCAL, false> : (sweep_tail_groups(c) ? k_step<PG_WM_GROUPS, true> : k_step<PG_WM_GROUPS, false>);
-    if (e0 || e1) hipExtLaunchKernelGGL(kern, dim3(md.nseg + 1), dim3(PG_BLK), 0, st, e0, e1, 0, md, ar, sp, sn, pr);
-    else hipLaunchKernelGGL(kern, dim3(md.nseg + 1), dim3(PG_BLK), 0, st, md, ar, sp, sn, pr);
+    const dim3 grid(1 + ((!local && sweep_tail_groups(c)) ? pg_scan_wgs(md.nseg) : 0) + md.nseg);
+    if (e0 || e1) hipExtLaunchKernelGGL(kern, grid, dim3(PG_BLK), 0, st, e0, e1, 0, md, ar, sp, sn, pr);
+    else hipLaunchKernelGGL(kern, grid, dim3(PG_BLK), 0, st, md, ar, sp, sn, pr);
     KCHK(c, "k_step");
     return PGAS_OK;
 }
@@ -1207,6 +1210,22 @@
     UpperHdr h;
     HIPCHK(c, hipMemcpy(&h, c->sb[c->md.T & 1].hdr, sizeof h, hipMemcpyDeviceToHost));
     *idx = h.final_idx;
+    int32_t gave_up = 0;
+    const int rc = pgas_scan_status(c, &gave_up, stream);
+    if (rc) return rc;
+    if (gave_up) FAIL(c, PGAS_E_STATE, "pgas_last_final_index: a group scan inside k_step gave up waiting for its segment partials; the sweep's results are not valid");
+    return PGAS_OK;
+}
+
+int pgas_scan_status(pgas_ctx* c, int32_t* gave_up, void* stream) {
+    if (!c) return PGAS_E_ARG;
+    if (!gave_up) FAIL(c, PGAS_E_ARG, "pgas_scan_status: NULL argument");
+    DeviceGuard guard(c->device);
+    HIPCHK(c, hipStreamSynchronize((hipStream_t)stream));
+    unsigned f[2] = {0u, 0u};
+    for (int i = 0; i < 2; ++i)
+        if (c->sb[i].scan_fail) HIPCHK(c, hipMemcpy(&f[i], c->sb[i].scan_fail, sizeof(unsigned), hipMemcpyDeviceToHost));
+    *gave_up = (f[0] | f[1]) ? 1 : 0;
     return PGAS_OK;
 }
 
@@ -1689,12 +1708,12 @@
 
 int pgas_detmath_eval(int32_t device, int32_t which, const double* x_dev, const double* y_dev, const uint32_t* w_dev, int64_t n, double* out0_dev,
                       double* out1_dev, uint32_t* outw_dev, void* stream) {
-    if (which < 0 || which > 8 || n < 0) return PGAS_E_ARG;
-    const bool words = which == 3 || which == 7;
+    if (which < 0 || which > 10 || n < 0) return PGAS_E_ARG;
+    const bool words = which == 3 || which == 7 || which == 9;
     if (words ? !w_dev : !x_dev) return PGAS_E_ARG;
     if ((which == 5 || which == 6) && !y_dev) return PGAS_E_ARG;
     if (which == 3 ? !outw_dev : !out0_dev) return PGAS_E_ARG;
-    if ((which == 2 || which == 7) && !out1_dev) return PGAS_E_ARG;
+    if ((which == 2 || which == 7 || which == 9 || which == 10) && !out1_dev) return PGAS_E_ARG;
     if (n == 0) return PGAS_OK;
     DeviceGuard guard(device);
     hipLaunchKernelGGL(k_detmath, dim3((unsigned)((n + 255) / 256)), dim3(256), 0, (hipStream_t)stream, which, x_dev, y_dev, w_dev, n, out0_dev, out1_dev, outw_dev);
diff --git a/bayesian-inference-with-explicit-and-implicit-prior-knowledge_amd/csrc/pgas_kernels.hip.h b/bayesian-inference-with-explicit-and-implicit-prior-knowledge_amd/csrc/pgas_kernels.hip.h
--- a/bayesian-inference-with-explicit-and-implicit-prior-knowledge_amd/csrc/pgas_kernels.hip.h
+++ b/bayesian-inference-with-explicit-and-implicit-prior-knowledge_amd/csrc/pgas_kernels.hip.h
@@ -164,7 +164,8 @@
     double* tab_m;
     double* grp_K;
     double* grp_T;
-    unsigned* grp_cnt;
+    unsigned long long* hand;
+    unsigned* scan_fail;
     UpperHdr* hdr;
 };
 
@@ -295,12 +296,15 @@
     double s0, c0, sd, cd;
 };
 
-template <int P, bool FAST = false>
+template <int P, bool GUARD>
+__device__ __forceinline__ void dev_sincospi_n(const double (&r)[P], double (&sp)[P], double (&cp)[P]);
+template <int P, bool FAST = false, bool SC = false>
 __device__ __forceinline__ void dim_start_n(const DevModel& md, int d, const double (&r)[P], DimStart (&ds)[P]) {
     double a[P], sv[P], cv[P];
 #pragma unroll
     for (int p = 0; p < P; ++p) a[p] = (double)md.j0[d] * r[p];
-    pgas_sincospi_n(a, sv, cv, P);
+    if constexpr (SC) dev_sincospi_n<P, true>(a, sv, cv);
+    else pgas_sincospi_n(a, sv, cv, P);
 #pragma unroll
     for (int p = 0; p < P; ++p) {
         ds[p].s0 = sv[p];
@@ -383,8 +387,9 @@
                 rin[p] = basis_arg<NX, DI, FAST>(md, x[p], ut);
                 rout[p] = basis_arg<NX, 0, FAST>(md, x[p], ut);
             }
-            dim_start_n<P, FAST>(md, DI, rin, din);
-            dim_start_n<P, FAST>(md, 0, rout, dout);
+            constexpr bool SC = FAST && D == 2;
+            dim_start_n<P, FAST, SC>(md, DI, rin, din);
+            dim_start_n<P, FAST, SC>(md, 0, rout, dout);
 #pragma unroll
             for (int p = 0; p < P; ++p) {
                 Cheb ci = cheb_init<FAST>(md, DI, din[p]);
@@ -786,6 +791,128 @@
     }
 }
 
+__device__ __forceinline__ double dev_fma_sc(double a, double b, double c_uniform) {
+#if defined(__HIP_DEVICE_COMPILE__)
+    double o;
+    asm("v_fma_f64 %0, %1, %2, %3" : "=v"(o) : "v"(a), "v"(b), "s"(c_uniform));
+    return o;
+#else
+    return PGAS_FMA(a, b, c_uniform);
+#endif
+}
+__device__ __forceinline__ double dev_div_normal(double x, double y) {
+    double r = __builtin_amdgcn_rcp(y);
+    double e = PGAS_FMA(-y, r, 1.0);
+    r = PGAS_FMA(r, e, r);
+    e = PGAS_FMA(-y, r, 1.0);
+    r = PGAS_FMA(r, e, r);
+    const double q = x * r;
+    const double d = PGAS_FMA(-y, q, x);
+    return PGAS_FMA(d, r, q);
+}
+__device__ __forceinline__ double dev_sqrt_normal(double x) {
+    const double y = __builtin_amdgcn_rsq(x);
+    const double s0 = x * y, h0 = y * 0.5;
+    const double r0 = PGAS_FMA(-h0, s0, 0.5);
+    const double s1 = PGAS_FMA(s0, r0, s0), h1 = PGAS_FMA(h0, r0, h0);
+    const double d0 = PGAS_FMA(-s1, s1, x);
+    const double s2 = PGAS_FMA(d0, h1, s1);
+    const double d1 = PGAS_FMA(-s2, s2, x);
+    return PGAS_FMA(d1, h1, s2);
+}
+template <int P, bool GUARD>
+__device__ __forceinline__ void dev_sincospi_n(const double (&r)[P], double (&sp)[P], double (&cp)[P]) {
+    const double PI_HI = 0x1.921fb54442d18p+1;
+    const double PI_LO = 0x1.1a62633145c07p-53;
+    const double S[8] = {0x1.aaec32af93359p-21, -0x1.6fadb9f155744p-16, 0x1.e8f434d018d63p-12, -0x1.e3074fde8871fp-8,
+                         0x1.50783487ee782p-4,  -0x1.32d2cce62bd86p-1,  0x1.466bc6775aae2p+1,  -0x1.4abbce625be53p+2};
+    const double Cc[8] = {0x1.20c62c2f2d7f5p-18, -0x1.b6e24f44b128fp-14, 0x1.f9d38a3763cc3p-10, -0x1.a6d1f2a204a8cp-6,
+                          0x1.e1f506891babbp-3,  -0x1.55d3c7e3cbffap+0,  0x1.03c1f081b5ac4p+2,  -0x1.3bd3cc9be45dep+2};
+    double nn[P], f[P], z[P], ps[P], pc[P];
+#pragma unroll
+    for (int i = 0; i < P; ++i) {
+        double rr = r[i];
+        if constexpr (GUARD) rr = (__builtin_fabs(r[i]) < 0x1p30) ? r[i] : 0.0;
+        nn[i] = __builtin_rint(rr + rr);
+        f[i] = PGAS_FMA(-0.5, nn[i], rr);
+        z[i] = f[i] * f[i];
+        ps[i] = -0x1.8a404211f9547p-26;
+        pc[i] = -0x1.2a0c591af8314p-23;
+    }
+#pragma unroll
+    for (int j = 0; j < 8; ++j)
+#pragma unroll
+        for (int i = 0; i < P; ++i) {
+            ps[i] = dev_fma_sc(ps[i], z[i], S[j]);
+            pc[i] = dev_fma_sc(pc[i], z[i], Cc[j]);
+        }
+#pragma unroll
+    for (int i = 0; i < P; ++i) {
+        const double fz = f[i] * z[i];
+        const double s = PGAS_FMA(f[i], PI_HI, PGAS_FMA(fz, ps[i], f[i] * PI_LO));
+        const double c = PGAS_FMA(z[i], pc[i], 1.0);
+        const uint32_t q = (uint32_t)(int32_t)nn[i];
+        uint64_t sb = pgas_d2bits((q & 1u) ? c : s);
+        uint64_t cb = pgas_d2bits((q & 1u) ? s : c);
+        sb ^= (uint64_t)(q & 2u) << 62;
+        cb ^= (uint64_t)((q + 1u) & 2u) << 62;
+        double so = pgas_bits2d(sb), co = pgas_bits2d(cb);
+        if constexpr (GUARD) {
+            if (r[i] != r[i]) {
+                so = r[i];
+                co = r[i];
+            }
+        }
+        sp[i] = so;
+        cp[i] = co;
+    }
+}
+template <int P>
+__device__ __forceinline__ void dev_normal_pair_n(const pgas_u32x4 (&w)[P], double (&z0)[P], double (&z1)[P]) {
+    const double LN2_HI = 0x1.62e42fee00000p-1;
+    const double LN2_LO = 0x1.a39ef35793c76p-33;
+    const double C[11] = {0x1.642c8590b2164p-4, 0x1.8618618618618p-4, 0x1.af286bca1af28p-4, 0x1.e1e1e1e1e1e1ep-4,
+                          0x1.1111111111111p-3, 0x1.3b13b13b13b14p-3, 0x1.745d1745d1746p-3, 0x1.c71c71c71c71cp-3,
+                          0x1.2492492492492p-2, 0x1.999999999999ap-2, 0x1.5555555555555p-1};
+    double ub2[P], f[P], k[P], s[P], z[P], R[P], lg[P], sn[P], cs[P];
+#pragma unroll
+    for (int i = 0; i < P; ++i) {
+        const uint32_t a_hi = w[i].v[1] >> 12, a_lo = (w[i].v[1] << 20) | (w[i].v[0] >> 12);
+        const uint32_t b_hi = w[i].v[3] >> 12, b_lo = (w[i].v[3] << 20) | (w[i].v[2] >> 12);
+        const double ua = __hiloint2double((int)(0x3ff00000u | a_hi), (int)a_lo) - 0x1.fffffffffffffp-1;
+        ub2[i] = __hiloint2double((int)(0x40000000u | b_hi), (int)b_lo) - 0x1.fffffffffffffp+0;
+        uint64_t b = pgas_d2bits(ua);
+        int32_t e = (int32_t)(b >> 52) - 1023;
+        const uint64_t mant = b & 0x000fffffffffffffULL;
+        const int big = mant > 0x6a09e667f3bcdULL;
+        e += big;
+        b = mant | (big ? 0x3fe0000000000000ULL : 0x3ff0000000000000ULL);
+        f[i] = pgas_bits2d(b) - 1.0;
+        k[i] = (double)e;
+        s[i] = dev_div_normal(f[i], 2.0 + f[i]);
+        z[i] = s[i] * s[i];
+        R[i] = 0x1.47ae147ae147bp-4;
+    }
+#pragma unroll
+    for (int j = 0; j < 11; ++j)
+#pragma unroll
+        for (int i = 0; i < P; ++i) R[i] = dev_fma_sc(R[i], z[i], C[j]);
+#pragma unroll
+    for (int i = 0; i < P; ++i) {
+        const double Rz = R[i] * z[i];
+        const double hfsq = 0.5 * f[i] * f[i];
+        const double t = PGAS_FMA(s[i], hfsq + Rz, k[i] * LN2_LO);
+        lg[i] = k[i] * LN2_HI - ((hfsq - t) - f[i]);
+    }
+    dev_sincospi_n<P, false>(ub2, sn, cs);
+#pragma unroll
+    for (int i = 0; i < P; ++i) {
+        const double rad = dev_sqrt_normal(-2.0 * lg[i]);
+        z0[i] = rad * cs[i];
+        z1[i] = rad * sn[i];
+    }
+}
+
 #define PG_QPLANE (PG_BLK + 8)
 __device__ __forceinline__ int q_slot(int i) { return (i & 3) * PG_QPLANE + (i >> 2); }
 struct ScanSmem {
@@ -797,7 +924,8 @@
 template <int NW, bool STORE_B = true, bool HANDOFF = false>
 __device__ __forceinline__ void segment_scan(ScanSmem& sm, const double (&lw)[NW][PG_PPT], int seg, int nsegp,
                                              uint64_t* __restrict__ cA, uint64_t* __restrict__ cB, double* __restrict__ segm,
-                                             uint64_t* __restrict__ segs) {
+                                             uint64_t* __restrict__ segs, unsigned long long* hand = nullptr, unsigned tag = 0) {
+    static_assert(!HANDOFF || NW == 2, "the hand-off granules carry both CDFs");
     const int tid = threadIdx.x, lane = tid & 63, wave = tid >> 6;
     double mx[NW];
 #pragma unroll
@@ -848,15 +976,29 @@
         if (lane == 63) sm.wtot[w][wave] = incl[w];
     }
     __syncthreads();
+    uint64_t offs[NW], tots[NW];
 #pragma unroll
     for (int w = 0; w < NW; ++w) {
-        uint64_t off = 0, tot = 0;
+        offs[w] = 0, tots[w] = 0;
 #pragma unroll
         for (int v = 0; v < PG_BLK / 64; ++v) {
             const uint64_t t = sm.wtot[w][v];
-            if (v < wave) off += t;
-            tot += t;
-        }
+            if (v < wave) offs[w] += t;
+            tots[w] += t;
+        }
+    }
+    if constexpr (HANDOFF) {
+        if (tid < 8) {
+            const bool hb = tid >> 2;
+            const uint64_t bits = (tid & 2) ? (hb ? tots[NW - 1] : tots[0]) : pgas_d2bits(hb ? mx[NW - 1] : mx[0]);
+            const uint32_t half = (tid & 1) ? (uint32_t)(bits >> 32) : (uint32_t)bits;
+            __hip_atomic_store(&hand[(size_t)seg * 8 + tid], ((unsigned long long)tag << 32) | half, __ATOMIC_RELAXED, __HIP_MEMORY_SCOPE_AGENT);
+        }
+    }
+#pragma unroll
+    for (int w = 0; w < NW; ++w) {
+        const uint64_t off = offs[w], tot = tots[w];
+        (void)tot;
         if (w == 0 || STORE_B) {
             const uint64_t base = off + incl[w] - loc[w][PG_PPT - 1];
             uint64_t* segc = (w == 0 ? cA : cB) + (size_t)seg * PGAS_SEG;
@@ -864,11 +1006,8 @@
             st_row16<PG_ST_C1>(dst, segc, 32u * tid, pg_nt_u2{base + loc[w][0], base + loc[w][1]}, PGAS_SEG * 8u);
             st_row16<PG_ST_C1>(dst + 1, segc, 32u * tid + 16u, pg_nt_u2{base + loc[w][2], base + loc[w][3]}, PGAS_SEG * 8u);
         }
-        if (tid == 0) {
-            if constexpr (HANDOFF) {
-                __hip_atomic_store(&segm[(size_t)w * nsegp + seg], mx[w], __ATOMIC_RELAXED, __HIP_MEMORY_SCOPE_AGENT);
-                __hip_atomic_store(&segs[(size_t)w * nsegp + seg], tot, __ATOMIC_RELAXED, __HIP_MEMORY_SCOPE_AGENT);
-            } else {
+        if constexpr (!HANDOFF) {
+            if (tid == 0) {
                 segm[(size_t)w * nsegp + seg] = mx[w];
                 segs[(size_t)w * nsegp + seg] = tot;
             }
@@ -1008,7 +1147,7 @@
     segment_scan<2>(sm, lw, seg, sb.nsegp, sb.c1, sb.c2, sb.segk_w, sb.segs_w);
 }
 
-template <int NX, int P>
+template <int NX, int P, bool SC = false>
 __device__ __forceinline__ void propagate_finish(const DevModel& md, const TransParams& tp, int t, uint64_t seed, const double (&rf)[NX],
                                                  const double* __restrict__ yt, int seg, int r0, const double (&aux)[P][NX],
                                                  double (&xn)[P][NX], double (&la)[P], double (&h)[P], double (&ln)[P]) {
@@ -1021,7 +1160,8 @@
             const int64_t pi = (int64_t)seg * PGAS_SEG + (r0 + p) * PG_BLK + tid;
             w[p] = pgas_rng_block(seed, PGAS_STREAM_PROP, 0u, (uint32_t)t, (uint64_t)(md.p0 + pi));
         }
-        pgas_normal_pair_n(w, z0, z1, P);
+        if constexpr (SC) dev_normal_pair_n<P>(w, z0, z1);
+        else pgas_normal_pair_n(w, z0, z1, P);
     }
 #pragma unroll
     for (int p = 0; p < P; ++p) {
@@ -1053,7 +1193,7 @@
                                                 const double (&xin)[P][NX], double (&xn)[P][NX], double (&la)[P], double (&h)[P], double (&ln)[P]) {
     double aux[P][NX];
     eval_mean<NX, D, JIN, P, J0T>(md, G, ut, xin, aux);
-    propagate_finish<NX, P>(md, tp, t, seed, rf, yt, seg, r0, aux, xn, la, h, ln);
+    propagate_finish<NX, P, (D == 2 && J0T > 0)>(md, tp, t, seed, rf, yt, seg, r0, aux, xn, la, h, ln);
 }
 
 template <int NX, int D, int JIN, int P, int J0T, int PPT, bool ONE, uint64_t MXD = 0>
diff --git a/bayesian-inference-with-explicit-and-implicit-prior-knowledge_amd/csrc/pgas_resample.hip.h b/bayesian-inference-with-explicit-and-implicit-prior-knowledge_amd/csrc/pgas_resample.hip.h
--- a/bayesian-inference-with-explicit-and-implicit-prior-knowledge_amd/csrc/pgas_resample.hip.h
+++ b/bayesian-inference-with-explicit-and-implicit-prior-knowledge_amd/csrc/pgas_resample.hip.h
@@ -80,21 +80,9 @@
     return __builtin_fmax(p.cp, p.E + p.sg * v);
 }
 
-__device__ __forceinline__ void group_records_wave(const ScanBufs& sb, int nseg, int cdf, int g, bool coherent) {
+__device__ __forceinline__ void group_records_from(const ScanBufs& sb, int nseg, int cdf, int g, double kk, uint64_t ss) {
     const int lane = threadIdx.x & 63;
     const int b = g * PG_GRP + lane;
-    double kk = -__builtin_inf();
-    uint64_t ss = 0;
-    if (b < nseg) {
-        const size_t at = partial_at(sb, cdf, b);
-        if (coherent) {
-            kk = __hip_atomic_load(&sb.segk[at], __ATOMIC_RELAXED, __HIP_MEMORY_SCOPE_AGENT);
-            ss = __hip_atomic_load(&sb.segs[at], __ATOMIC_RELAXED, __HIP_MEMORY_SCOPE_AGENT);
-        } else {
-            kk = sb.segk[at];
-            ss = sb.segs[at];
-        }
-    }
     double e, sc, m, Kg;
     group_scan_wave(kk, ss, e, sc, m, Kg);
     const int nb = nseg - g * PG_GRP < PG_GRP ? nseg - g * PG_GRP : PG_GRP;
@@ -110,13 +98,24 @@
         sb.grp_T[cdf * PG_MAX_GRP + g] = Tg;
     }
 }
+__device__ __forceinline__ void group_records_wave(const ScanBufs& sb, int nseg, int cdf, int g) {
+    const int b = g * PG_GRP + (threadIdx.x & 63);
+    double kk = -__builtin_inf();
+    uint64_t ss = 0;
+    if (b < nseg) {
+        const size_t at = partial_at(sb, cdf, b);
+        kk = sb.segk[at];
+        ss = sb.segs[at];
+    }
+    group_records_from(sb, nseg, cdf, g, kk, ss);
+}
 
 __global__ __launch_bounds__(256) void k_groups(int nseg, int ncdf, ScanBufs sb) {
     __builtin_amdgcn_s_setprio(3);
     const int n1 = (nseg + PG_GRP - 1) / PG_GRP;
     const int w = blockIdx.x * 4 + (threadIdx.x >> 6);
     if (w >= n1 * ncdf) return;
-    group_records_wave(sb, nseg, w / n1, w % n1, false);
+    group_records_wave(sb, nseg, w / n1, w % n1);
 }
 
 #define PG_WM_GROUPS 0
@@ -725,6 +724,48 @@
     return cdf_count_wg<LOCAL>(sm, sb, pr, 1, nseg, N, U, nullptr, nullptr, &in);
 }
 
+__host__ __device__ inline int pg_scan_wgs(int nseg) { return (2 * ((nseg + PG_GRP - 1) / PG_GRP) + 3) / 4; }
+#ifndef PG_SCAN_SPINS
+#define PG_SCAN_SPINS (1 << 23)
+#endif
+__device__ __forceinline__ void scanner_groups(const ScanBufs& sb, int nseg, unsigned tag) {
+    const int lane = threadIdx.x & 63;
+    const int n1 = (nseg + PG_GRP - 1) / PG_GRP;
+    const int w = ((int)blockIdx.x - 1) * (PG_BLK / 64) + (threadIdx.x >> 6);
+    if (w >= 2 * n1) return;
+    const int cdf = w / n1, g = w % n1;
+    const int b = g * PG_GRP + lane;
+    const bool exists = b < nseg;
+    const unsigned long long* gr = sb.hand + ((size_t)(exists ? b : g * PG_GRP) * 2 + cdf) * 4;
+    unsigned v[4] = {0u, 0u, 0u, 0u};
+    bool ok = !exists;
+    for (int spins = 0;; ++spins) {
+        if (!ok) {
+            bool m = true;
+#pragma unroll
+            for (int k = 0; k < 4; ++k) {
+                const unsigned long long x = __hip_atomic_load(gr + k, __ATOMIC_RELAXED, __HIP_MEMORY_SCOPE_AGENT);
+                v[k] = (unsigned)x;
+                m = m && (unsigned)(x >> 32) == tag;
+            }
+            ok = m;
+        }
+        if (__all(ok)) break;
+        if (spins >= PG_SCAN_SPINS) {
+            if (lane == 0) __hip_atomic_store(sb.scan_fail, 1u, __ATOMIC_RELAXED, __HIP_MEMORY_SCOPE_AGENT);
+            return;
+        }
+        __builtin_amdgcn_s_sleep(8);
+    }
+    __builtin_amdgcn_s_setprio(3);
+    const double kk = exists ? pgas_bits2d(((uint64_t)v[1] << 32) | v[0]) : -__builtin_inf();
+    const uint64_t ss = exists ? (((uint64_t)v[3] << 32) | v[2]) : 0ull;
+    if (exists) {
+        sb.segk_w[(size_t)cdf * sb.nsegp + b] = kk;
+        sb.segs_w[(size_t)cdf * sb.nsegp + b] = ss;
+    }
+    group_records_from(sb, nseg, cdf, g, kk, ss);
+}
 #ifndef PG_STEP_OCC
 #define PG_STEP_OCC 4
 #endif
@@ -746,7 +787,15 @@
                                __HIP_MEMORY_SCOPE_AGENT);
         return;
     }
-    const int seg = blockIdx.x - 1;
+    int seg = blockIdx.x - 1;
+    if constexpr (TAIL) {
+        const int nscan = pg_scan_wgs(md.nseg);
+        if (seg < nscan) {
+            if (ar.mode & PG_RS_SCAN) scanner_groups(sb_next, md.nseg, tag);
+            return;
+        }
+        seg -= nscan;
+    }
     const int64_t base_i = (int64_t)seg * PGAS_SEG;
     PG_STAMP(0);
     double lnv[PG_PPT] = {0.0, 0.0, 0.0, 0.0};
@@ -864,27 +913,8 @@
             }
         }
         PG_STAMP(6);
-        segment_scan<2, false, TAIL>(sm.u.scan, lw, seg, sb_next.nsegp, sb_next.c1, sb_next.c2, sb_next.segk_w, sb_next.segs_w);
+        segment_scan<2, false, TAIL>(sm.u.scan, lw, seg, sb_next.nsegp, sb_next.c1, sb_next.c2, sb_next.segk_w, sb_next.segs_w, sb_next.hand, tag);
         PG_STAMP(8);
-        if constexpr (TAIL) {
-            if (tid < 64) {
-                const int g = seg / PG_GRP;
-                const int nb = md.nseg - g * PG_GRP < PG_GRP ? md.nseg - g * PG_GRP : PG_GRP;
-                unsigned arrived = 0;
-                if (tid == 0) {
-                    asm volatile("s_waitcnt vmcnt(0)" ::: "memory");
-                    arrived = __hip_atomic_fetch_add(&sb_next.grp_cnt[g], 1u, __ATOMIC_RELAXED, __HIP_MEMORY_SCOPE_AGENT);
-                }
-                arrived = __builtin_amdgcn_readfirstlane(arrived);
-                if (arrived == (unsigned)(nb - 1)) {
-                    __builtin_amdgcn_fence(__ATOMIC_ACQUIRE, "agent");
-                    asm volatile("s_waitcnt vmcnt(0)" ::: "memory");
-                    group_records_wave(sb_next, md.nseg, 0, g, true);
-                    group_records_wave(sb_next, md.nseg, 1, g, true);
-                    if (tid == 0) __hip_atomic_store(&sb_next.grp_cnt[g], 0u, __ATOMIC_RELAXED, __HIP_MEMORY_SCOPE_AGENT);
-                }
-            }
-        }
     }
     if (ar.mode & PG_RS_SEARCH) store_trace();
     PG_STAMP(7);
@@ -928,6 +958,22 @@
         uint64_t qv[1];
         dev_exp_q51_n<1>(xv, qv);
         o0[i] = (double)qv[0];
+        break;
+    }
+    case 9: {
+        const pgas_u32x4 r[1] = {{{w[6 * i], w[6 * i + 1], w[6 * i + 2], w[6 * i + 3]}}};
+        double a[1], b[1];
+        dev_normal_pair_n<1>(r, a, b);
+        o0[i] = a[0];
+        o1[i] = b[0];
+        break;
+    }
+    case 10: {
+        const double xv[1] = {x[i]};
+        double sv[1], cv[1];
+        dev_sincospi_n<1, true>(xv, sv, cv);
+        o0[i] = sv[0];
+        o1[i] = cv[0];
         break;
     }
     default: break;
diff --git a/include/pgas_hip.h b/include/pgas_hip.h
--- a/include/pgas_hip.h
+++ b/include/pgas_hip.h
@@ -70,6 +70,7 @@
 int pgas_trace_row(pgas_ctx* ctx, int32_t kind, int32_t t, void** row_dev);
 
 int pgas_last_final_index(pgas_ctx* ctx, int64_t* idx, void* stream);
+int pgas_scan_status(pgas_ctx* ctx, int32_t* gave_up, void* stream);
 
 int pgas_set_profiling(pgas_ctx* ctx, int32_t on);
 int pgas_get_profile(pgas_ctx* ctx, int64_t* resample_launches, double* resample_ms, int64_t* propagate_launches,
```

Result: faster. 35.80 billion particle-steps/s (median of 6 runs) (+2.0%).
